# dkazanc/ToMoBAR

Hardware: AMD Instinct MI355X
Metric: fista_os_iterations_per_sec (higher is better)
Workload: dtype f32; 1 GPU; FISTA-OS(12 subsets)+PD_TV(30 inner, f32 duals), 900 angles, 1024 slices of 1024^2 per GPU; slab-iterations/s over 1 z-slab(s) (BASELINE configs[2]); slices_per_gpu=1024, n=1024, angles=900, os_number=12, method=FISTA, output_finite=True, input=analytic ellipsoid line integrals + Poisson noise (I0 2e4, peak attenuation 3), oversubscribed=False

## Files before the change

include/tomo_mi355x.h:

```cpp
#ifndef TOMO_MI355X_H
#define TOMO_MI355X_H

#include <stddef.h>
#include <stdint.h>

#ifdef __cplusplus
extern "C" {
#endif

#define TOMO_ABI_VERSION 10

enum {
    TOMO_OK = 0,
    TOMO_E_INVALID = 1,
    TOMO_E_RUNTIME = 2,
    TOMO_E_NOMEM = 3,
    TOMO_E_NODEVICE = 4
};

#define TOMO_FLAG_LERP8 1u

enum { TOMO_FID_LS = 0, TOMO_FID_PWLS = 1, TOMO_FID_KL = 2, TOMO_FID_RATIO = 3 };

typedef struct tomo_ctx tomo_ctx;

typedef struct {
    float cs, sn;
    float cor;
    float slope;
    float inv;
    float scale;
    int32_t dirx;
    int32_t src;
} tomo_angle_t;

int tomo_abi_version(void);
const char *tomo_build_flavour(void);
const char *tomo_last_error(void);
int tomo_device_count(int *count);

int tomo_ctx_create(int device, int nz, int n, int nu, int na, const double *angles_host,
                    const double *cor_host, int cor_stride, int os_number, unsigned flags,
                    tomo_ctx **out);
int tomo_ctx_destroy(tomo_ctx *ctx);
int tomo_ctx_os_number(const tomo_ctx *ctx);
int tomo_ctx_num_bins(const tomo_ctx *ctx);
int tomo_ctx_newind_table(const tomo_ctx *ctx, int64_t *out_host);
int tomo_ctx_subset_size(const tomo_ctx *ctx, int subset);
int tomo_ctx_angle_table(const tomo_ctx *ctx, int subset, tomo_angle_t *out_host, int capacity);
int tomo_ctx_release_scratch(tomo_ctx *ctx);
const char *tomo_ctx_kernel_path(const tomo_ctx *ctx, const char *op);

int tomo_fp3d(tomo_ctx *ctx, int subset, const float *vol_dev, float *sino_dev, void *stream);
int tomo_bp3d(tomo_ctx *ctx, int subset, const float *sino_dev, float *vol_dev, void *stream);

#define TOMO_GATHERED_B 1
#define TOMO_GATHERED_W 2
int tomo_fp3d_residual(tomo_ctx *ctx, int subset, const float *vol_dev, const float *b_dev,
                       const float *w_dev, int gathered, int fidelity, float *res_dev, void *stream);

enum { TOMO_ROBUST_NONE = 0, TOMO_ROBUST_HUBER = 1, TOMO_ROBUST_STUDENTST = 2 };
int tomo_fp3d_residual_robust(tomo_ctx *ctx, int subset, const float *vol_dev, const float *b_dev, const float *w_dev,
                              int gathered, int fidelity, int robust, float delta, float *res_dev, void *stream);
int tomo_sino_robust(float *res_dev, size_t count, int robust, float delta, void *stream);

int tomo_fp3d_residual_ring(tomo_ctx *ctx, int subset, const float *vol_dev, const float *b_full_dev,
                            const float *ring_dev, float ring_scale, float *res_dev, void *stream);
int tomo_ring_gh_reduce(float *res_dev, const float *w_full_dev, const int *src_dev, int nz, int na_s, int na_full,
                        int nu, const float *rx_dev, float l_inv, float *r_out_dev, void *stream);
int tomo_swls_apply(float *res_dev, const float *w_full_dev, const int *src_dev, int nz, int na_s, int na_full, int nu,
                    float beta, void *stream);
int tomo_ring_gh_update(float *r_dev, float *r_old_dev, float *rx_dev, float lambda, float beta, size_t count,
                        void *stream);

int tomo_shift_rows(const float *in_dev, float *out_dev, int nz, int na, int nu, const float *shift_dev, float sign,
                    void *stream);
int tomo_sino_residual(const float *ax_dev, const float *b_full_dev, const float *w_full_dev, const int *src_dev, int nz,
                       int na_s, int na_full, int nu, int gathered, int fidelity, float *res_dev, void *stream);
int tomo_sino_add_ring(float *res_dev, const float *ring_dev, float ring_scale, int nz, int na_s, int nu, void *stream);

int tomo_bp3d_fista(tomo_ctx *ctx, int subset, const float *res_dev, const float *xt_dev,
                    float *xout_dev, float l_inv, int nonneg, void *stream);
int tomo_bp3d_fista_momentum(tomo_ctx *ctx, int subset, const float *res_dev, float *xt_dev,
                             float *xold_x_dev, float l_inv, float beta, int nonneg, void *stream);
int tomo_bp3d_admm(tomo_ctx *ctx, int subset, const float *res_dev, float *z_dev, const float *x_dev,
                   const float *u_dev, float *zu_out_dev, float tau, float rho, int relax_on,
                   float one_minus_alpha, float alpha, int nonneg, void *stream);

int tomo_bp3d_matched(tomo_ctx *ctx, int subset, const float *sino_dev, float *vol_dev, void *stream);
int tomo_bp3d_matched_fista(tomo_ctx *ctx, int subset, const float *res_dev, const float *xt_dev,
                            float *xout_dev, float l_inv, int nonneg, void *stream);
int tomo_bp3d_matched_fista_momentum(tomo_ctx *ctx, int subset, const float *res_dev, float *xt_dev,
                                     float *xold_x_dev, float l_inv, float beta, int nonneg, void *stream);
int tomo_bp3d_matched_admm(tomo_ctx *ctx, int subset, const float *res_dev, float *z_dev, const float *x_dev,
                           const float *u_dev, float *zu_out_dev, float tau, float rho, int relax_on,
                           float one_minus_alpha, float alpha, int nonneg, void *stream);

enum { TOMO_RESIDUAL_PLANAR = 0, TOMO_RESIDUAL_ZQUAD = 1 };
int tomo_ctx_set_residual_layout(tomo_ctx *ctx, int layout);
int tomo_ctx_residual_layout(const tomo_ctx *ctx);
size_t tomo_ctx_residual_elems(const tomo_ctx *ctx, int subset);

int tomo_momentum(const float *x_dev, const float *xold_dev, float *xt_dev, float beta, size_t count, void *stream);
int tomo_momentum_transposed(tomo_ctx *ctx, const float *x_dev, const float *xold_dev, float *xt_dev, float beta,
                             void *stream);
int tomo_ctx_invalidate(tomo_ctx *ctx);
int tomo_admm_dual(float *u_dev, const float *z_dev, const float *x_dev, size_t count, void *stream);
int tomo_axpby(float a, const float *x_dev, float b, float *y_dev, size_t count, void *stream);
int tomo_scale(float a, const float *x_dev, float *y_dev, size_t count, void *stream);
int tomo_clamp_min(float *x_dev, float lo, size_t count, void *stream);
int tomo_mul(const float *x_dev, float *y_dev, size_t count, void *stream);
int tomo_recip_safe(const float *x_dev, float *y_dev, size_t count, void *stream);
int tomo_fill(float *x_dev, float value, size_t count, void *stream);
int tomo_norm2(const float *x_dev, size_t count, double *out_host, void *stream);
int tomo_dot(const float *x_dev, const float *y_dev, size_t count, double *out_host, void *stream);
int tomo_max(const float *x_dev, size_t count, float *out_host, void *stream);
int tomo_rel_change(const float *x_dev, const float *ref_dev, float *keep_dev, size_t count, double out_host[2], void *stream);
int tomo_pwls_weights(const float *b_dev, float *w_dev, size_t count, void *stream);
int tomo_pwls_max(const float *b_dev, size_t count, float *out_host, void *stream);
int tomo_pwls_weights_scaled(const float *b_dev, float *w_dev, size_t count, float wmax, void *stream);
int tomo_diag_stream(const float *const *in_dev, int nin, float *const *out_dev, int nout, size_t count,
                     int vec, int grid, void *stream);

int tomo_pad_edge(const float *in_dev, float *out_dev, int rows, int nu0, int pad, void *stream);
int tomo_crop_center(const float *in_dev, float *out_dev, int nz, int n, int m, void *stream);
int tomo_circ_mask(float *vol_dev, int nz, int n, double radius, void *stream);
int tomo_permute3(const float *in_dev, float *out_dev, int d0, int d1, int d2,
                  int64_t s0, int64_t s1, int64_t s2, void *stream);

int tomo_pdtv(int device, const float *in_dev, float *out_dev, int dx, int dy, int dz, int nd,
              float sigma, float tau, float lt, float theta, int iters, int methodTV, int nonneg,
              int half, void *stream);
int tomo_roftv(int device, const float *in_dev, float *out_dev, int dx, int dy, int dz, int nd,
               float lambda, float tau, int iters, int half, void *stream);
int tomo_pdtv_tol(int device, const float *in_dev, float *out_dev, int dx, int dy, int dz, int nd,
                  float sigma, float tau, float lt, float theta, int iters, int methodTV, int nonneg,
                  int half, double tol, int *iters_done, double *last_rel_change, void *stream);
int tomo_roftv_tol(int device, const float *in_dev, float *out_dev, int dx, int dy, int dz, int nd,
                   float lambda, float tau, int iters, int half, double tol, int *iters_done,
                   double *last_rel_change, void *stream);
int tomo_pdtv_slices(int device, const float *in_dev, float *out_dev, int dx, int dy, int nslices, float sigma,
                     float tau, float lt, float theta, int iters, int methodTV, int nonneg, int half, double tol,
                     int *iters_done, double *last_rel_change, void *stream);
int tomo_roftv_slices(int device, const float *in_dev, float *out_dev, int dx, int dy, int nslices, float lambda,
                      float tau, int iters, int half, double tol, int *iters_done, double *last_rel_change,
                      void *stream);
size_t tomo_pdtv_slices_scratch_bytes(int dx, int dy, int nslices, int half);
size_t tomo_roftv_slices_scratch_bytes(int dx, int dy, int nslices);
int tomo_tgv(int device, const float *in_dev, float *out_dev, int dx, int dy, int dz, int nd,
             float lambda, float alpha1, float alpha0, float tau, float sigma, int iters,
             double tol, int *iters_done, double *last_rel_change, void *stream);
enum { TOMO_NDF_HUBER = 0, TOMO_NDF_PM = 1, TOMO_NDF_TUKEY = 2 };
int tomo_ndf(int device, const float *in_dev, float *out_dev, int dx, int dy, int dz, int nd,
             float lambda, float sigma, float tau, int penalty, int iters,
             double tol, int *iters_done, double *last_rel_change, void *stream);
int tomo_diff4th(int device, const float *in_dev, float *out_dev, int dx, int dy, int dz, int nd,
                 float lambda, float sigma, float tau, int iters,
                 double tol, int *iters_done, double *last_rel_change, void *stream);
int tomo_llt_rof(int device, const float *in_dev, float *out_dev, int dx, int dy, int dz, int nd,
                 float lambda_rof, float lambda_llt, float tau, int iters,
                 double tol, int *iters_done, double *last_rel_change, void *stream);
size_t tomo_wavelet_scratch_bytes(int dx, int dy, int dz, int nd);
int tomo_wavelet_shrink(int device, const float *in_dev, float *out_dev, const float *mix_dev, int dx, int dy, int dz,
                        int nd, float threshold, void *stream);
int tomo_wavelet_forward(int device, const float *in_dev, float *pyramid_dev, int dx, int dy, int dz, int nd,
                         float threshold, void *stream);
int tomo_wavelet_inverse(int device, float *pyramid_dev, float *out_dev, const float *mix_dev, int dx, int dy, int dz,
                         int nd, void *stream);
size_t tomo_nltv_scratch_bytes(int dx, int dy, int dz, int nd);
int tomo_patch_select(int device, const float *in_dev, uint16_t *hi_dev, uint16_t *hj_dev, float *w_dev,
                      int dx, int dy, int dz, int nd, int search, int patch, int neighbours, float h, void *stream);
int tomo_nltv(int device, const float *in_dev, float *out_dev, const uint16_t *hi_dev, const uint16_t *hj_dev,
              const float *w_dev, int dx, int dy, int dz, int nd, int neighbours, float lambda, int iters,
              double tol, int *iters_done, double *last_rel_change, void *stream);
size_t tomo_pdtv_scratch_bytes(int dx, int dy, int dz, int nd, int half);
size_t tomo_roftv_scratch_bytes(int dx, int dy, int dz, int nd);
size_t tomo_tgv_scratch_bytes(int dx, int dy, int dz, int nd);
size_t tomo_ndf_scratch_bytes(int dx, int dy, int dz, int nd);
size_t tomo_diff4th_scratch_bytes(int dx, int dy, int dz, int nd);
size_t tomo_llt_rof_scratch_bytes(int dx, int dy, int dz, int nd);
int tomo_release_scratch(int device);
int tomo_reserve_scratch(int device, size_t bytes, void *stream);
int tomo_set_placement_tries(int tries);
int tomo_placement_tries(void);
int tomo_placed_scratch(int device, int slot, size_t bytes, void *stream, void **out_dev);
int tomo_placement_last(size_t *bytes, int *chosen, double *scores_GBps, int capacity);
int tomo_placement_last_fast(void);

int tomo_pdtv_iter_slab(int device, const float *in_dev, const float *u_in_dev, float *u_out_dev,
                        const void *p_in_dev[3], void *p_out_dev[3], int dx, int dy, int nz_local,
                        int has_lo, int has_hi, float sigma, float tau, float lt, float theta,
                        int methodTV, int nonneg, int half, void *stream);
int tomo_pdtv_multi_slab_range(int device, const float *in_dev, const float *u_in_dev, float *u_out_dev,
                               const void *p_in_dev[3], void *p_out_dev[3], int dx, int dy, int nz_local,
                               int lo_planes, int hi_planes, int z_begin, int z_end, int k, float sigma, float tau,
                               float lt, float theta, int methodTV, int nonneg, int half, void *stream);
int tomo_roftv_iter_slab_range(int device, const float *in_dev, const float *u_in_dev, float *u_out_dev,
                               int dx, int dy, int nz_local, int lo_planes, int hi_planes, int z_begin, int z_end,
                               float lambda, float tau, int half, void *stream);
int tomo_ndf_iter_slab_range(int device, const float *in_dev, const float *u_in_dev, float *u_out_dev,
                             int dx, int dy, int nz_local, int lo_planes, int hi_planes, int z_begin, int z_end,
                             float lambda, float sigma, float tau, int penalty, void *stream);
int tomo_diff4th_iter_slab_range(int device, const float *in_dev, const float *u_in_dev, float *u_out_dev,
                                 int dx, int dy, int nz_local, int lo_planes, int hi_planes, int z_begin, int z_end,
                                 float lambda, float sigma, float tau, void *stream);
int tomo_llt_rof_iter_slab_range(int device, const float *in_dev, const float *u_in_dev, float *u_out_dev,
                                 int dx, int dy, int nz_local, int lo_planes, int hi_planes, int z_begin, int z_end,
                                 float lambda_rof, float lambda_llt, float tau, void *stream);

size_t tomo_halo_staging_bytes(const size_t *bytes, int nblocks);
int tomo_halo_pack(const void *const *src_dev, const size_t *bytes, int nblocks, void *staging_dev, void *stream);
int tomo_halo_unpack(const void *staging_dev, void *const *dst_dev, const size_t *bytes, int nblocks, void *stream);
int tomo_halo_pack2(const void *const *src_down_dev, const size_t *bytes_down, int nblocks_down, void *msg_down_dev,
                    const void *const *src_up_dev, const size_t *bytes_up, int nblocks_up, void *msg_up_dev, void *stream);
int tomo_halo_pull2(const void *msg_down_dev, void *const *dst_down_dev, const size_t *bytes_down, int nblocks_down,
                    const void *msg_up_dev, void *const *dst_up_dev, const size_t *bytes_up, int nblocks_up, void *stream);
int tomo_ipc_region_create(int device, size_t bytes, void **base_dev, unsigned char handle[64]);
int tomo_ipc_region_open(int device, const unsigned char handle[64], void **mapped_dev);
int tomo_ipc_region_close(void *mapped_dev);
int tomo_ipc_region_destroy(void *base_dev);
int tomo_pdtv_iters_per_launch(int half);
int tomo_pdtv_launch_plan(int iters, int nd, int dz, int *k_out, int capacity);

int tomo_fbp_filter(int device, float *data_dev, size_t rows, int nu, float cutoff, float multiplier, void *stream);

int tomo_fourier_inv(int device, const float *data_dev, float *out_dev, int nz, int out_z, int nproj, int raw_n,
                     int n, int ne, int unpad_m, int out_size, const float *w_host, const float *theta_host,
                     int m, float mu, int center_size, void *stream);

int tomo_set_variant(const char *kernel, int variant);

int tomo_profile_enable(int on);
int tomo_profile_read(const char *kernel, long long *launches, double *total_ms);

int tomo_host_bp2d(const float *sino_host, float *img_host, int n, int nu, int na, const double *angles_host, double cor);
int tomo_host_fp2d(const float *img_host, float *sino_host, int n, int nu, int na, const double *angles_host, double cor);

#ifdef __cplusplus
}
#endif
#endif
```

tomobar_amd/_lib.py:

```python

from __future__ import annotations

import contextvars
import ctypes as C
import os
import threading

_HERE = os.path.dirname(os.path.abspath(__file__))
LIB_PATH = os.path.join(_HERE, "libtomo_mi355x.so")

OK, E_INVALID, E_RUNTIME, E_NOMEM, E_NODEVICE = 0, 1, 2, 3, 4
ABI_VERSION = 10
FLAG_LERP8 = 1
FID = {"LS": 0, "PWLS": 1, "KL": 2, "RATIO": 3}
ROBUST = {None: 0, "huber": 1, "studentst": 2}
RESIDUAL_LAYOUT = {"planar": 0, "zquad": 1}
NDF_PENALTY = {"Huber": 0, "PM": 1, "Tukey": 2}


def ndf_penalty_id(penalty_type) -> int:
    if penalty_type not in NDF_PENALTY:
        raise ValueError(f"unknown NDF penalty {penalty_type!r}: Huber, PM and Tukey are supported")
    return NDF_PENALTY[penalty_type]


class AngleRecord(C.Structure):
    _fields_ = [("cs", C.c_float), ("sn", C.c_float), ("cor", C.c_float), ("slope", C.c_float),
                ("inv", C.c_float), ("scale", C.c_float), ("dirx", C.c_int32), ("src", C.c_int32)]


_vp, _i, _f, _d, _sz = C.c_void_p, C.c_int, C.c_float, C.c_double, C.c_size_t

SIGNATURES = {
    "tomo_abi_version": (_i, []),
    "tomo_build_flavour": (C.c_char_p, []),
    "tomo_last_error": (C.c_char_p, []),
    "tomo_device_count": (_i, [C.POINTER(_i)]),
    "tomo_ctx_create": (_i, [_i, _i, _i, _i, _i, C.POINTER(_d), C.POINTER(_d), _i, _i, C.c_uint, C.POINTER(_vp)]),
    "tomo_ctx_destroy": (_i, [_vp]),
    "tomo_ctx_os_number": (_i, [_vp]),
    "tomo_ctx_num_bins": (_i, [_vp]),
    "tomo_ctx_newind_table": (_i, [_vp, C.POINTER(C.c_int64)]),
    "tomo_ctx_subset_size": (_i, [_vp, _i]),
    "tomo_ctx_angle_table": (_i, [_vp, _i, C.POINTER(AngleRecord), _i]),
    "tomo_ctx_release_scratch": (_i, [_vp]),
    "tomo_ctx_kernel_path": (C.c_char_p, [_vp, C.c_char_p]),
    "tomo_fp3d": (_i, [_vp, _i, _vp, _vp, _vp]),
    "tomo_bp3d": (_i, [_vp, _i, _vp, _vp, _vp]),
    "tomo_fp3d_residual": (_i, [_vp, _i, _vp, _vp, _vp, _i, _i, _vp, _vp]),
    "tomo_fp3d_residual_robust": (_i, [_vp, _i, _vp, _vp, _vp, _i, _i, _i, _f, _vp, _vp]),
    "tomo_sino_robust": (_i, [_vp, _sz, _i, _f, _vp]),
    "tomo_fp3d_residual_ring": (_i, [_vp, _i, _vp, _vp, _vp, _f, _vp, _vp]),
    "tomo_ring_gh_reduce": (_i, [_vp, _vp, _vp, _i, _i, _i, _i, _vp, _f, _vp, _vp]),
    "tomo_swls_apply": (_i, [_vp, _vp, _vp, _i, _i, _i, _i, _f, _vp]),
    "tomo_ring_gh_update": (_i, [_vp, _vp, _vp, _f, _f, _sz, _vp]),
    "tomo_shift_rows": (_i, [_vp, _vp, _i, _i, _i, _vp, _f, _vp]),
    "tomo_sino_add_ring": (_i, [_vp, _vp, _f, _i, _i, _i, _vp]),
    "tomo_sino_residual": (_i, [_vp, _vp, _vp, _vp, _i, _i, _i, _i, _i, _i, _vp, _vp]),
    "tomo_bp3d_fista": (_i, [_vp, _i, _vp, _vp, _vp, _f, _i, _vp]),
    "tomo_bp3d_fista_momentum": (_i, [_vp, _i, _vp, _vp, _vp, _f, _f, _i, _vp]),
    "tomo_bp3d_admm": (_i, [_vp, _i, _vp, _vp, _vp, _vp, _vp, _f, _f, _i, _f, _f, _i, _vp]),
    "tomo_bp3d_matched": (_i, [_vp, _i, _vp, _vp, _vp]),
    "tomo_bp3d_matched_fista": (_i, [_vp, _i, _vp, _vp, _vp, _f, _i, _vp]),
    "tomo_bp3d_matched_fista_momentum": (_i, [_vp, _i, _vp, _vp, _vp, _f, _f, _i, _vp]),
    "tomo_bp3d_matched_admm": (_i, [_vp, _i, _vp, _vp, _vp, _vp, _vp, _f, _f, _i, _f, _f, _i, _vp]),
    "tomo_ctx_set_residual_layout": (_i, [_vp, _i]),
    "tomo_ctx_residual_layout": (_i, [_vp]),
    "tomo_ctx_residual_elems": (_sz, [_vp, _i]),
    "tomo_momentum": (_i, [_vp, _vp, _vp, _f, _sz, _vp]),
    "tomo_momentum_transposed": (_i, [_vp, _vp, _vp, _vp, _f, _vp]),
    "tomo_ctx_invalidate": (_i, [_vp]),
    "tomo_admm_dual": (_i, [_vp, _vp, _vp, _sz, _vp]),
    "tomo_axpby": (_i, [_f, _vp, _f, _vp, _sz, _vp]),
    "tomo_scale": (_i, [_f, _vp, _vp, _sz, _vp]),
    "tomo_clamp_min": (_i, [_vp, _f, _sz, _vp]),
    "tomo_mul": (_i, [_vp, _vp, _sz, _vp]),
    "tomo_recip_safe": (_i, [_vp, _vp, _sz, _vp]),
    "tomo_fill": (_i, [_vp, _f, _sz, _vp]),
    "tomo_norm2": (_i, [_vp, _sz, C.POINTER(_d), _vp]),
    "tomo_dot": (_i, [_vp, _vp, _sz, C.POINTER(_d), _vp]),
    "tomo_max": (_i, [_vp, _sz, C.POINTER(_f), _vp]),
    "tomo_rel_change": (_i, [_vp, _vp, _vp, _sz, C.POINTER(_d), _vp]),
    "tomo_pwls_weights": (_i, [_vp, _vp, _sz, _vp]),
    "tomo_pwls_max": (_i, [_vp, _sz, C.POINTER(_f), _vp]),
    "tomo_pwls_weights_scaled": (_i, [_vp, _vp, _sz, _f, _vp]),
    "tomo_diag_stream": (_i, [C.POINTER(_vp), _i, C.POINTER(_vp), _i, _sz, _i, _i, _vp]),
    "tomo_pad_edge": (_i, [_vp, _vp, _i, _i, _i, _vp]),
    "tomo_crop_center": (_i, [_vp, _vp, _i, _i, _i, _vp]),
    "tomo_circ_mask": (_i, [_vp, _i, _i, _d, _vp]),
    "tomo_permute3": (_i, [_vp, _vp, _i, _i, _i, C.c_int64, C.c_int64, C.c_int64, _vp]),
    "tomo_pdtv": (_i, [_i, _vp, _vp, _i, _i, _i, _i, _f, _f, _f, _f, _i, _i, _i, _i, _vp]),
    "tomo_roftv": (_i, [_i, _vp, _vp, _i, _i, _i, _i, _f, _f, _i, _i, _vp]),
    "tomo_pdtv_tol": (_i, [_i, _vp, _vp, _i, _i, _i, _i, _f, _f, _f, _f, _i, _i, _i, _i, _d, C.POINTER(_i), C.POINTER(_d), _vp]),
    "tomo_roftv_tol": (_i, [_i, _vp, _vp, _i, _i, _i, _i, _f, _f, _i, _i, _d, C.POINTER(_i), C.POINTER(_d), _vp]),
    "tomo_pdtv_scratch_bytes": (_sz, [_i, _i, _i, _i, _i]),
    "tomo_roftv_scratch_bytes": (_sz, [_i, _i, _i, _i]),
    "tomo_pdtv_slices": (_i, [_i, _vp, _vp, _i, _i, _i, _f, _f, _f, _f, _i, _i, _i, _i, _d, C.POINTER(_i), C.POINTER(_d), _vp]),
    "tomo_roftv_slices": (_i, [_i, _vp, _vp, _i, _i, _i, _f, _f, _i, _i, _d, C.POINTER(_i), C.POINTER(_d), _vp]),
    "tomo_pdtv_slices_scratch_bytes": (_sz, [_i, _i, _i, _i]),
    "tomo_roftv_slices_scratch_bytes": (_sz, [_i, _i, _i]),
    "tomo_tgv": (_i, [_i, _vp, _vp, _i, _i, _i, _i, _f, _f, _f, _f, _f, _i, _d, C.POINTER(_i), C.POINTER(_d), _vp]),
    "tomo_tgv_scratch_bytes": (_sz, [_i, _i, _i, _i]),
    "tomo_ndf": (_i, [_i, _vp, _vp, _i, _i, _i, _i, _f, _f, _f, _i, _i, _d, C.POINTER(_i), C.POINTER(_d), _vp]),
    "tomo_ndf_scratch_bytes": (_sz, [_i, _i, _i, _i]),
    "tomo_diff4th": (_i, [_i, _vp, _vp, _i, _i, _i, _i, _f, _f, _f, _i, _d, C.POINTER(_i), C.POINTER(_d), _vp]),
    "tomo_diff4th_scratch_bytes": (_sz, [_i, _i, _i, _i]),
    "tomo_llt_rof": (_i, [_i, _vp, _vp, _i, _i, _i, _i, _f, _f, _f, _i, _d, C.POINTER(_i), C.POINTER(_d), _vp]),
    "tomo_llt_rof_scratch_bytes": (_sz, [_i, _i, _i, _i]),
    "tomo_wavelet_scratch_bytes": (_sz, [_i, _i, _i, _i]),
    "tomo_wavelet_shrink": (_i, [_i, _vp, _vp, _vp, _i, _i, _i, _i, _f, _vp]),
    "tomo_wavelet_forward": (_i, [_i, _vp, _vp, _i, _i, _i, _i, _f, _vp]),
    "tomo_wavelet_inverse": (_i, [_i, _vp, _vp, _vp, _i, _i, _i, _i, _vp]),
    "tomo_nltv_scratch_bytes": (_sz, [_i, _i, _i, _i]),
    "tomo_patch_select": (_i, [_i, _vp, _vp, _vp, _vp, _i, _i, _i, _i, _i, _i, _i, _f, _vp]),
    "tomo_nltv": (_i, [_i, _vp, _vp, _vp, _vp, _vp, _i, _i, _i, _i, _i, _f, _i, _d, C.POINTER(_i), C.POINTER(_d), _vp]),
    "tomo_release_scratch": (_i, [_i]),
    "tomo_reserve_scratch": (_i, [_i, _sz, _vp]),
    "tomo_set_placement_tries": (_i, [_i]),
    "tomo_placement_tries": (_i, []),
    "tomo_placement_last_fast": (_i, []),
    "tomo_placed_scratch": (_i, [_i, _i, _sz, _vp, C.POINTER(_vp)]),
    "tomo_placement_last": (_i, [C.POINTER(C.c_size_t), C.POINTER(_i), C.POINTER(C.c_double), _i]),
    "tomo_pdtv_iter_slab": (_i, [_i, _vp, _vp, _vp, C.POINTER(_vp), C.POINTER(_vp), _i, _i, _i, _i, _i,
                                 _f, _f, _f, _f, _i, _i, _i, _vp]),
    "tomo_pdtv_multi_slab_range": (_i, [_i, _vp, _vp, _vp, C.POINTER(_vp), C.POINTER(_vp), _i, _i, _i, _i, _i, _i, _i, _i,
                                        _f, _f, _f, _f, _i, _i, _i, _vp]),
    "tomo_roftv_iter_slab_range": (_i, [_i, _vp, _vp, _vp, _i, _i, _i, _i, _i, _i, _i, _f, _f, _i, _vp]),
    "tomo_ndf_iter_slab_range": (_i, [_i, _vp, _vp, _vp, _i, _i, _i, _i, _i, _i, _i, _f, _f, _f, _i, _vp]),
    "tomo_diff4th_iter_slab_range": (_i, [_i, _vp, _vp, _vp, _i, _i, _i, _i, _i, _i, _i, _f, _f, _f, _vp]),
    "tomo_llt_rof_iter_slab_range": (_i, [_i, _vp, _vp, _vp, _i, _i, _i, _i, _i, _i, _i, _f, _f, _f, _vp]),
    "tomo_halo_staging_bytes": (_sz, [C.POINTER(_sz), _i]),
    "tomo_halo_pack": (_i, [C.POINTER(_vp), C.POINTER(_sz), _i, _vp, _vp]),
    "tomo_halo_unpack": (_i, [_vp, C.POINTER(_vp), C.POINTER(_sz), _i, _vp]),
    "tomo_halo_pack2": (_i, [C.POINTER(_vp), C.POINTER(_sz), _i, _vp, C.POINTER(_vp), C.POINTER(_sz), _i, _vp, _vp]),
    "tomo_halo_pull2": (_i, [_vp, C.POINTER(_vp), C.POINTER(_sz), _i, _vp, C.POINTER(_vp), C.POINTER(_sz), _i, _vp]),
    "tomo_ipc_region_create": (_i, [_i, _sz, C.POINTER(_vp), C.POINTER(C.c_ubyte)]),
    "tomo_ipc_region_open": (_i, [_i, C.POINTER(C.c_ubyte), C.POINTER(_vp)]),
    "tomo_ipc_region_close": (_i, [_vp]),
    "tomo_ipc_region_destroy": (_i, [_vp]),
    "tomo_pdtv_iters_per_launch": (_i, [_i]),
    "tomo_pdtv_launch_plan": (_i, [_i, _i, _i, C.POINTER(_i), _i]),
    "tomo_fbp_filter": (_i, [_i, _vp, _sz, _i, _f, _f, _vp]),
    "tomo_fourier_inv": (_i, [_i, _vp, _vp, _i, _i, _i, _i, _i, _i, _i, _i, _vp, _vp, _i, _f, _i, _vp]),
    "tomo_host_bp2d": (_i, [_vp, _vp, _i, _i, _i, C.POINTER(_d), _d]),
    "tomo_host_fp2d": (_i, [_vp, _vp, _i, _i, _i, C.POINTER(_d), _d]),
    "tomo_set_variant": (_i, [C.c_char_p, _i]),
    "tomo_profile_enable": (_i, [_i]),
    "tomo_profile_read": (_i, [C.c_char_p, C.POINTER(C.c_longlong), C.POINTER(_d)]),
}

LIB_PATHS = {"shipped": LIB_PATH, "dev": os.path.join(_HERE, "libtomo_mi355x_dev.so")}
_handles = {}
_DEFAULT_FLAVOUR = "dev" if os.environ.get("TOMO_MI355X_FLAVOUR", "shipped") == "dev" else "shipped"
_flavour_var = contextvars.ContextVar("tomo_mi355x_flavour", default=_DEFAULT_FLAVOUR)


class TomoRuntimeError(RuntimeError):
    pass


def _load(flavour: str):
    path = LIB_PATHS[flavour]
    if not os.path.exists(path):
        raise ImportError(
            f"{path} not found: the HIP extension is required (no CPU fallback). "
            f"Build it with `make -C tomobar_amd/csrc{' dev' if flavour == 'dev' else ''}` or `__graft_entry__.build()`.")
    handle = C.CDLL(path)
    missing = [name for name in SIGNATURES if not hasattr(handle, name)]
    if missing:
        raise ImportError(f"{path} is stale: it does not export {missing[:4]}{'...' if len(missing) > 4 else ''}; "
                          "rebuild it (make -C tomobar_amd/csrc all)")
    for name, (res, args) in SIGNATURES.items():
        fn = getattr(handle, name)
        fn.restype = res
        fn.argtypes = args
    if handle.tomo_abi_version() != ABI_VERSION:
        raise ImportError(f"{os.path.basename(path)} has ABI version {handle.tomo_abi_version()}, this package binds "
                          f"version {ABI_VERSION}: rebuild it (make -C tomobar_amd/csrc all)")
    if handle.tomo_build_flavour().decode() != flavour:
        raise ImportError(f"{path} reports flavour {handle.tomo_build_flavour().decode()!r}, expected {flavour!r}")
    return handle


_load_lock = threading.Lock()


def lib():
    name = _flavour_var.get()
    h = _handles.get(name)
    if h is None:
        with _load_lock:
            h = _handles.get(name)
            if h is None:
                h = _handles[name] = _load(name)
    return h


def flavour() -> str:
    return _flavour_var.get()


class use_flavour:

    def __init__(self, name: str):
        if name not in LIB_PATHS:
            raise ValueError(f"unknown library flavour {name!r}")
        self.name = name
        self._token = None

    def __enter__(self):
        self._token = _flavour_var.set(self.name)
        return lib()

    def __exit__(self, *exc):
        if self._token is not None:
            _flavour_var.reset(self._token)
            self._token = None
        return False

    enter, exit = __enter__, __exit__


def check(rc: int, handle=None):
    if rc == OK:
        return
    msg = (handle or lib()).tomo_last_error().decode("utf-8", "replace")
    if rc == E_INVALID:
        raise ValueError(msg)
    if rc == E_NOMEM:
        raise MemoryError(msg)
    raise TomoRuntimeError(msg)
```

tomobar_amd/csrc/proj_kernels.hip:

```cpp
#include "tomo_common.h"

#include <algorithm>
#include <atomic>
#include <cmath>
#include <map>
#include <mutex>
#include <numeric>
#include <string>
#include <type_traits>

namespace {

template <bool LERP8>
__device__ __forceinline__ float lerp_w(float f, float fl)
{
    float w = f - fl;
    if (LERP8) w = rintf(w * 256.0f) * (1.0f / 256.0f);
    return w;
}

__device__ __forceinline__ float robust_weight(float r, int mode, float delta)
{
    if (mode == TOMO_ROBUST_HUBER) {
        const float ar = fabsf(r);
        if (ar > delta) r = (delta / ar) * r;
    } else if (mode == TOMO_ROBUST_STUDENTST) {
        r = (2.0f / (delta * delta + r * r)) * r;
    }
    return r;
}

enum { EPI_PLAIN = 0, EPI_FISTA = 1, EPI_FISTA_MOM = 2, EPI_ADMM = 3 };

struct BpArgs {
    const float *sino;
    int zquad;
    const tomo_angle_t *tab;
    int nz, n, nu, na;
    float *vol;
    const float *xt;
    float *xout;
    float *xt_out;
    const float *xold;
    float s0, s1, s2, s3;
    int nonneg, relax_on;
    int ntx, nty, nzb;
    int epi_aligned;
    int device;
    std::string *path;
};

template <int EPI>
__device__ __forceinline__ void bp_epilogue(const BpArgs &a, size_t idx, float g)
{
    if (EPI == EPI_PLAIN) {
        a.vol[idx] = g;
    } else if (EPI == EPI_FISTA) {
        float x = a.xt[idx] - a.s0 * g;
        if (a.nonneg) x = x < 0.0f ? 0.0f : x;
        a.xout[idx] = x;
    } else if (EPI == EPI_FISTA_MOM) {
        float x = a.xt[idx] - a.s0 * g;
        if (a.nonneg) x = x < 0.0f ? 0.0f : x;
        const float xo = a.xold[idx];
        a.xout[idx] = x;
        a.xt_out[idx] = x + a.s1 * (x - xo);
    } else {
        const float z0 = a.xout[idx], u = a.xold[idx];
        const float ga = a.s1 * ((z0 - a.xt[idx]) + u);
        float z = z0 - a.s0 * (g + ga);
        if (a.nonneg) z = z < 0.0f ? 0.0f : z;
        if (a.relax_on) z = a.s2 * z0 + a.s3 * z;
        a.xout[idx] = z;
        a.xt_out[idx] = z + u;
    }
}

template <int EPI>
__device__ __forceinline__ void bp_epilogue4(const BpArgs &a, size_t idx, float4 g)
{
#ifndef TOMO_BP_EPI_TEMPORAL
    typedef float v4 __attribute__((ext_vector_type(4)));
    auto ld4 = [&](const float *p) {
        const v4 t = __builtin_nontemporal_load(reinterpret_cast<const v4 *>(p + idx));
        return make_float4(t.x, t.y, t.z, t.w);
    };
    auto st4 = [&](float *p, float4 v) { __builtin_nontemporal_store(v4{v.x, v.y, v.z, v.w}, reinterpret_cast<v4 *>(p + idx)); };
#else
    auto ld4 = [&](const float *p) { return *reinterpret_cast<const float4 *>(p + idx); };
    auto st4 = [&](float *p, float4 v) { *reinterpret_cast<float4 *>(p + idx) = v; };
#endif
    const float gv[4] = {g.x, g.y, g.z, g.w};
    if (EPI == EPI_PLAIN) {
        st4(a.vol, g);
    } else if (EPI == EPI_FISTA) {
        const float4 t4 = ld4(a.xt);
        const float tv[4] = {t4.x, t4.y, t4.z, t4.w};
        float o[4];
#pragma unroll
        for (int k = 0; k < 4; ++k) {
            float x = tv[k] - a.s0 * gv[k];
            if (a.nonneg) x = x < 0.0f ? 0.0f : x;
            o[k] = x;
        }
        st4(a.xout, make_float4(o[0], o[1], o[2], o[3]));
    } else if (EPI == EPI_FISTA_MOM) {
        const float4 t4 = ld4(a.xt), o4 = ld4(a.xold);
        const float tv[4] = {t4.x, t4.y, t4.z, t4.w}, ov[4] = {o4.x, o4.y, o4.z, o4.w};
        float o[4], m[4];
#pragma unroll
        for (int k = 0; k < 4; ++k) {
            float x = tv[k] - a.s0 * gv[k];
            if (a.nonneg) x = x < 0.0f ? 0.0f : x;
            o[k] = x;
            m[k] = x + a.s1 * (x - ov[k]);
        }
        st4(a.xout, make_float4(o[0], o[1], o[2], o[3]));
        st4(a.xt_out, make_float4(m[0], m[1], m[2], m[3]));
    } else {
        const float4 z4 = ld4(a.xout), u4 = ld4(a.xold), t4 = ld4(a.xt);
        const float zv[4] = {z4.x, z4.y, z4.z, z4.w}, uv[4] = {u4.x, u4.y, u4.z, u4.w}, tv[4] = {t4.x, t4.y, t4.z, t4.w};
        float o[4], m[4];
#pragma unroll
        for (int k = 0; k < 4; ++k) {
            const float ga = a.s1 * ((zv[k] - tv[k]) + uv[k]);
            float z = zv[k] - a.s0 * (gv[k] + ga);
            if (a.nonneg) z = z < 0.0f ? 0.0f : z;
            if (a.relax_on) z = a.s2 * zv[k] + a.s3 * z;
            o[k] = z;
            m[k] = z + uv[k];
        }
        st4(a.xout, make_float4(o[0], o[1], o[2], o[3]));
        st4(a.xt_out, make_float4(m[0], m[1], m[2], m[3]));
    }
}

template <int EPI, bool LERP8>
__global__ __launch_bounds__(256) void bp_direct_kernel(BpArgs a)
{
    constexpr int ZB = 4;
    const int ix = blockIdx.x * 64 + (threadIdx.x & 63);
    const int iy = blockIdx.y * 4 + (threadIdx.x >> 6);
    const int z0 = blockIdx.z * ZB;
    if (ix >= a.n || iy >= a.n) return;
    const float half_n = 0.5f * (float)a.n - 0.5f, half_u = 0.5f * (float)a.nu - 0.5f;
    const float xw = (float)ix - half_n, yw = (float)iy - half_n;
    float acc[ZB] = {0.0f, 0.0f, 0.0f, 0.0f};
    const size_t zstride = (size_t)a.na * a.nu;
    for (int k = 0; k < a.na; ++k) {
        const tomo_angle_t t = a.tab[k];
        const float off = half_u - t.cor;
        const float f = fmaf(xw, t.cs, fmaf(yw, t.sn, off));
        const float fl = floorf(f);
        const float w = lerp_w<LERP8>(f, fl), omw = 1.0f - w;
        const int i0 = (int)fl;
        const bool ok0 = (i0 >= 0) && (i0 < a.nu), ok1 = (i0 + 1 >= 0) && (i0 + 1 < a.nu);
        if (a.zquad) {
            const float4 *row4 = reinterpret_cast<const float4 *>(a.sino) + ((size_t)(z0 >> 2) * a.na + k) * a.nu;
            const float4 zero4 = make_float4(0.0f, 0.0f, 0.0f, 0.0f);
            const float4 q0 = ok0 ? row4[i0] : zero4, q1 = ok1 ? row4[i0 + 1] : zero4;
            const float t0[ZB] = {q0.x, q0.y, q0.z, q0.w}, t1[ZB] = {q1.x, q1.y, q1.z, q1.w};
#pragma unroll
            for (int zz = 0; zz < ZB; ++zz) {
                acc[zz] = fmaf(omw, t0[zz], acc[zz]);
                acc[zz] = fmaf(w, t1[zz], acc[zz]);
            }
            continue;
        }
        const float *row = a.sino + ((size_t)z0 * a.na + k) * a.nu;
#pragma unroll
        for (int zz = 0; zz < ZB; ++zz) {
            const bool zok = z0 + zz < a.nz;
            const float s0 = (ok0 && zok) ? row[zz * zstride + i0] : 0.0f;
            const float s1 = (ok1 && zok) ? row[zz * zstride + i0 + 1] : 0.0f;
            acc[zz] = fmaf(omw, s0, acc[zz]);
            acc[zz] = fmaf(w, s1, acc[zz]);
        }
    }
#pragma unroll
    for (int zz = 0; zz < ZB; ++zz)
        if (z0 + zz < a.nz) bp_epilogue<EPI>(a, ((size_t)(z0 + zz) * a.n + iy) * a.n + ix, acc[zz]);
}

constexpr int BP_TX = 64, BP_TY = 8, BP_RY = 2, BP_ZQ = 4, BP_AB = 8, BP_PITCH = 72;

template <int EPI, bool LERP8>
__global__ __launch_bounds__(256) void bp_tiled_kernel(BpArgs a)
{
    __shared__ float4 tile[BP_AB][BP_ZQ][BP_PITCH];
    __shared__ int umin_s[BP_AB];

    const int ntiles = a.ntx * a.nty;
    const int b = blockIdx.x, xcd = b & 7, q = b >> 3;
    const int per_xcd = (a.nzb * ntiles + 7) >> 3;
    const int wi = xcd * per_xcd + q;
    if (wi >= a.nzb * ntiles) return;
    const int zb = wi / ntiles;
    const int tid = wi % ntiles;
    const int tx0 = (tid % a.ntx) * BP_TX, ty0 = (tid / a.ntx) * BP_TY;
    const int z0 = zb * (4 * BP_ZQ);

    const int lane = threadIdx.x & 63, wave = threadIdx.x >> 6;
    const int ix = tx0 + lane;
    const float half_n = 0.5f * (float)a.n - 0.5f, half_u = 0.5f * (float)a.nu - 0.5f;
    const float xw = (float)ix - half_n;
    float yw[BP_RY];
#pragma unroll
    for (int r = 0; r < BP_RY; ++r) yw[r] = (float)(ty0 + wave * BP_RY + r) - half_n;

    float acc[BP_RY][4 * BP_ZQ];
#pragma unroll
    for (int r = 0; r < BP_RY; ++r)
#pragma unroll
        for (int j = 0; j < 4 * BP_ZQ; ++j) acc[r][j] = 0.0f;

    const size_t zstride = (size_t)a.na * a.nu;
    for (int a0 = 0; a0 < a.na; a0 += BP_AB) {
        const int nb = min(BP_AB, a.na - a0);
        __syncthreads();
        if ((int)threadIdx.x < nb) {
            const tomo_angle_t t = a.tab[a0 + threadIdx.x];
            const float off = half_u - t.cor;
            const float x0 = (float)tx0 - half_n, x1 = (float)(tx0 + BP_TX - 1) - half_n;
            const float y0 = (float)ty0 - half_n, y1 = (float)(ty0 + BP_TY - 1) - half_n;
            const float f00 = fmaf(x0, t.cs, fmaf(y0, t.sn, off)), f10 = fmaf(x1, t.cs, fmaf(y0, t.sn, off));
            const float f01 = fmaf(x0, t.cs, fmaf(y1, t.sn, off)), f11 = fmaf(x1, t.cs, fmaf(y1, t.sn, off));
            umin_s[threadIdx.x] = (int)floorf(fminf(fminf(f00, f10), fminf(f01, f11)));
        }
        __syncthreads();
        for (int item = threadIdx.x; item < nb * BP_ZQ * BP_PITCH; item += 256) {
            const int j = item % BP_PITCH;
            const int zq = (item / BP_PITCH) % BP_ZQ;
            const int aa = item / (BP_PITCH * BP_ZQ);
            const int u = umin_s[aa] + j;
            float4 v = make_float4(0.0f, 0.0f, 0.0f, 0.0f);
            if (u >= 0 && u < a.nu) {
                const int z = z0 + zq * 4;
                const float *p = a.sino + ((size_t)z * a.na + (a0 + aa)) * a.nu + u;
                if (z + 0 < a.nz) v.x = p[0];
                if (z + 1 < a.nz) v.y = p[zstride];
                if (z + 2 < a.nz) v.z = p[2 * zstride];
                if (z + 3 < a.nz) v.w = p[3 * zstride];
            }
            tile[aa][zq][j] = v;
        }
        __syncthreads();
        for (int aa = 0; aa < nb; ++aa) {
            const tomo_angle_t t = a.tab[a0 + aa];
            const float off = half_u - t.cor;
            const int um = umin_s[aa];
#pragma unroll
            for (int r = 0; r < BP_RY; ++r) {
                const float f = fmaf(xw, t.cs, fmaf(yw[r], t.sn, off));
                const float fl = floorf(f);
                const float w = lerp_w<LERP8>(f, fl), omw = 1.0f - w;
                const int idx = (int)fl - um;
#pragma unroll
                for (int zq = 0; zq < BP_ZQ; ++zq) {
                    const float4 s0 = tile[aa][zq][idx];
                    const float4 s1 = tile[aa][zq][idx + 1];
                    float *c = &acc[r][zq * 4];
                    c[0] = fmaf(omw, s0.x, c[0]); c[0] = fmaf(w, s1.x, c[0]);
                    c[1] = fmaf(omw, s0.y, c[1]); c[1] = fmaf(w, s1.y, c[1]);
                    c[2] = fmaf(omw, s0.z, c[2]); c[2] = fmaf(w, s1.z, c[2]);
                    c[3] = fmaf(omw, s0.w, c[3]); c[3] = fmaf(w, s1.w, c[3]);
                }
            }
        }
    }
    if (ix < a.n) {
#pragma unroll
        for (int r = 0; r < BP_RY; ++r) {
            const int iy = ty0 + wave * BP_RY + r;
            if (iy < a.n) {
#pragma unroll
                for (int j = 0; j < 4 * BP_ZQ; ++j)
                    if (z0 + j < a.nz) bp_epilogue<EPI>(a, ((size_t)(z0 + j) * a.n + iy) * a.n + ix, acc[r][j]);
            }
        }
    }
}

#include "bp_brick.inl"

__global__ __launch_bounds__(256) void sino_to_quad_kernel(const float *__restrict__ in, float4 *__restrict__ out, int nz, size_t row)
{
    const size_t i = (size_t)blockIdx.x * 256 + threadIdx.x;
    const int z = 4 * (int)blockIdx.y;
    if (i >= row) return;
    const float *p = in + (size_t)z * row + i;
    float4 v;
    v.x = p[0];
    v.y = z + 1 < nz ? p[row] : 0.0f;
    v.z = z + 2 < nz ? p[2 * row] : 0.0f;
    v.w = z + 3 < nz ? p[3 * row] : 0.0f;
    out[(size_t)blockIdx.y * row + i] = v;
}

constexpr size_t BP_RELAY_MAX_BYTES = (size_t)16 << 30;
constexpr int BP_RELAY_DEVICES = 64, BP_RELAY_RETRY = 64;
struct bp_relay_state { std::atomic<size_t> refused{~(size_t)0}; std::atomic<unsigned> skipped{0}; };
bp_relay_state g_bp_relay[BP_RELAY_DEVICES];

template <int EPI>
int bp_launch(BpArgs a, bool lerp8, hipStream_t st)
{
    TOMO_ON_DEVICE(a.device);
    tomo_prof_scope prof(PROF_BP, st, 1);
    {
        uintptr_t bits = 0;
        if (EPI == EPI_PLAIN) bits |= (uintptr_t)a.vol;
        else bits |= (uintptr_t)a.xt | (uintptr_t)a.xout;
        if (EPI == EPI_FISTA_MOM || EPI == EPI_ADMM) bits |= (uintptr_t)a.xt_out | (uintptr_t)a.xold;
        a.epi_aligned = (bits & 15) == 0;
    }
    if (EPI == EPI_PLAIN) a.zquad = 0;
    if (a.zquad && (((uintptr_t)a.sino) & 15) != 0)
        return tomo_fail(TOMO_E_INVALID, "the quad-interleaved residual must be 16-byte aligned");
    bool relaid = false;
    if (g_variant_bp == 0 && !a.zquad && (long)a.na * a.nu < (1L << 25) && a.na > 0) {
        const size_t row = (size_t)a.na * a.nu, nq = (size_t)ceil_div(a.nz, 4), bytes = nq * row * 16;
        void *q = nullptr;
        bp_relay_state &rs = g_bp_relay[a.device >= 0 && a.device < BP_RELAY_DEVICES ? a.device : 0];
        bool have = bytes <= BP_RELAY_MAX_BYTES && nq <= 65535;
        if (have && bytes >= rs.refused.load() && (rs.skipped.fetch_add(1) + 1) % BP_RELAY_RETRY != 0) have = false;
        if (have) {
            const int rc = tomo_arena_get(a.device, st, ARENA_BPQ, bytes, &q);
            if (rc == TOMO_E_NOMEM) {
                rs.refused.store(std::min(rs.refused.load(), bytes));
                tomo_warn_once("bp_relay", "back projection: no memory for the quad-interleaved relay of a planar sinogram, "
                                           "running the planar staging (slower; asked again every 64th call and after tomo_release_scratch)");
                have = false;
            } else if (rc != TOMO_OK) {
                return rc;
            } else {
                rs.refused.store(~(size_t)0);
            }
        }
        if (have) {
            sino_to_quad_kernel<<<dim3((unsigned)((row + 255) / 256), (unsigned)nq), 256, 0, st>>>(a.sino, (float4 *)q, a.nz, row);
            TOMO_LAUNCH_CHECK();
            a.sino = (const float *)q;
            a.zquad = 1;
            relaid = true;
        }
    }
    const bool brick_ok = (long)a.na * a.nu < (a.zquad ? (1L << 25) : (1L << 27));
    const int variant = g_variant_bp == 3 ? 0 : g_variant_bp;
    if (variant == 1 || (variant == 0 && !brick_ok)) {
        if (variant == 0)
            tomo_warn_once("bp_direct", "back projection: angles x detector >= 2^27 samples per slice, falling back to "
                                        "the direct (no LDS) kernel (about 3.5x slower)");
        if (a.path) *a.path = "direct(no LDS)";
        dim3 grid(ceil_div(a.n, 64), ceil_div(a.n, 4), ceil_div(a.nz, 4));
        if (lerp8) bp_direct_kernel<EPI, true><<<grid, 256, 0, st>>>(a);
        else bp_direct_kernel<EPI, false><<<grid, 256, 0, st>>>(a);
    } else if (variant == 0) {
        if (a.path) *a.path = "brick(32x16x16)";
        a.ntx = ceil_div(a.n, BB_TX);
        a.nty = ceil_div(a.n, BB_TY);
        a.nzb = ceil_div(a.nz, 4 * BB_ZQ);
        const long blocks = 8L * (((long)a.nzb * a.ntx * a.nty + 7) / 8);
        if (blocks > 0x7fffffffL) return tomo_fail(TOMO_E_INVALID, "volume too large for one BP launch");
        if (a.zquad) {
            if (a.path) *a.path = relaid ? "brick(32x16x16, planar sinogram re-laid quad-interleaved, LDS-DMA staging)"
                                         : "brick(32x16x16, quad-interleaved residual, LDS-DMA staging)";
            if (lerp8) bp_brick_kernel<EPI, true, true><<<(unsigned)blocks, 256, 0, st>>>(a);
            else bp_brick_kernel<EPI, false, true><<<(unsigned)blocks, 256, 0, st>>>(a);
            TOMO_LAUNCH_CHECK();
            return TOMO_OK;
        }
        if (lerp8) bp_brick_kernel<EPI, true><<<(unsigned)blocks, 256, 0, st>>>(a);
        else bp_brick_kernel<EPI, false><<<(unsigned)blocks, 256, 0, st>>>(a);
    }
#if TOMO_DEV
    else {
        if (a.zquad) return tomo_fail(TOMO_E_INVALID, "bp variant 2 reads the planar residual layout only");
        if (a.path) *a.path = "tiled(64x8x16)";
        a.ntx = ceil_div(a.n, BP_TX);
        a.nty = ceil_div(a.n, BP_TY);
        a.nzb = ceil_div(a.nz, 4 * BP_ZQ);
        const long blocks = 8L * (((long)a.nzb * a.ntx * a.nty + 7) / 8);
        if (blocks > 0x7fffffffL) return tomo_fail(TOMO_E_INVALID, "volume too large for one BP launch");
        if (lerp8) bp_tiled_kernel<EPI, true><<<(unsigned)blocks, 256, 0, st>>>(a);
        else bp_tiled_kernel<EPI, false><<<(unsigned)blocks, 256, 0, st>>>(a);
    }
#endif
    TOMO_LAUNCH_CHECK();
    return TOMO_OK;
}

struct FpArgs {
    const float *vol;
    const float *volT;
    const tomo_angle_t *tab;
    int nz, n, nu, na, na_full;
    float *out;
    const float *b;
    const float *w;
    const float *ring;
    float ring_scale;
    int fidelity;
    int gathered;
    int zquad;
    int robust;
    float rdelta;
};

template <class Args>
__device__ __forceinline__ float fp_residual_value(const Args &a, float val, int z, int k_a, int src, int iu)
{
    const size_t gi = ((size_t)z * a.na + k_a) * a.nu + iu;
    const size_t fi = ((size_t)z * a.na_full + src) * a.nu + iu;
    const float bv = a.b[(a.gathered & TOMO_GATHERED_B) ? gi : fi];
    if (a.fidelity == TOMO_FID_KL || a.fidelity == TOMO_FID_RATIO) {
        const float ax = val < 1e-8f ? 1e-8f : val;
        const float q = bv / ax;
        return (a.fidelity == TOMO_FID_KL) ? 1.0f - q : q;
    }
    val = val - bv;
    if (a.ring) val = val + a.ring_scale * a.ring[(size_t)z * a.nu + iu];
    if (a.w) val = val * a.w[(a.gathered & TOMO_GATHERED_W) ? gi : fi];
    return robust_weight(val, a.robust, a.rdelta);
}

__global__ __launch_bounds__(256) void transpose_inplane_kernel(const float *__restrict__ in, float *__restrict__ out, int n)
{
    __shared__ float t[32][33];
    const size_t zoff = (size_t)blockIdx.z * n * n;
    const int bx = blockIdx.x * 32, by = blockIdx.y * 32;
    const int lx = threadIdx.x & 31, ly = threadIdx.x >> 5;
    for (int r = ly; r < 32; r += 8) {
        const int x = bx + lx, y = by + r;
        t[r][lx] = (x < n && y < n) ? in[zoff + (size_t)y * n + x] : 0.0f;
    }
    __syncthreads();
    for (int r = ly; r < 32; r += 8) {
        const int y = by + lx, x = bx + r;
        if (x < n && y < n) out[zoff + (size_t)x * n + y] = t[lx][r];
    }
}

__global__ __launch_bounds__(256) void momentum_transpose_kernel(const float *__restrict__ x, const float *__restrict__ xold,
                                                                float *__restrict__ xt, float *__restrict__ xt_T, float beta, int n)
{
    __shared__ float t[32][33];
    const size_t zoff = (size_t)blockIdx.z * n * n;
    const int bx = blockIdx.x * 32, by = blockIdx.y * 32;
    const int lx = threadIdx.x & 31, ly = threadIdx.x >> 5;
    for (int r = ly; r < 32; r += 8) {
        const int xx = bx + lx, yy = by + r;
        float v = 0.0f;
        if (xx < n && yy < n) {
            const size_t i = zoff + (size_t)yy * n + xx;
            const float a = x[i];
            v = a + beta * (a - xold[i]);
            xt[i] = v;
        }
        t[r][lx] = v;
    }
    __syncthreads();
    for (int r = ly; r < 32; r += 8) {
        const int yy = by + lx, xx = bx + r;
        if (xx < n && yy < n) xt_T[zoff + (size_t)xx * n + yy] = t[lx][r];
    }
}

typedef float glue_v4 __attribute__((ext_vector_type(4)));
__device__ __forceinline__ float4 nt_ld4(const float *p)
{
    const glue_v4 v = __builtin_nontemporal_load(reinterpret_cast<const glue_v4 *>(p));
    return make_float4(v.x, v.y, v.z, v.w);
}
__device__ __forceinline__ void nt_st4(float *p, float4 v)
{
    __builtin_nontemporal_store(glue_v4{v.x, v.y, v.z, v.w}, reinterpret_cast<glue_v4 *>(p));
}
template <bool MOMENTUM>
__global__ __launch_bounds__(256) void transpose64_kernel(const float *__restrict__ x, const float *__restrict__ xold,
                                                          float *__restrict__ xt, float *__restrict__ xt_T, float beta, int n)
{
    __shared__ float t[64][65];
    const size_t zoff = (size_t)blockIdx.z * n * n;
    const int bx = blockIdx.x * 64, by = blockIdx.y * 64;
    const int c4 = (threadIdx.x & 15) * 4, r0 = threadIdx.x >> 4;
#pragma unroll
    for (int k = 0; k < 4; ++k) {
        const int r = r0 + 16 * k;
        const int xx = bx + c4, yy = by + r;
        float4 v = make_float4(0.0f, 0.0f, 0.0f, 0.0f);
        if (xx < n && yy < n) {
            const size_t i = zoff + (size_t)yy * n + xx;
            const float4 a = nt_ld4(x + i);
            if (MOMENTUM) {
                const float4 o = nt_ld4(xold + i);
                v.x = a.x + beta * (a.x - o.x); v.y = a.y + beta * (a.y - o.y);
                v.z = a.z + beta * (a.z - o.z); v.w = a.w + beta * (a.w - o.w);
                nt_st4(xt + i, v);
            } else {
                v = a;
            }
        }
        t[r][c4] = v.x; t[r][c4 + 1] = v.y; t[r][c4 + 2] = v.z; t[r][c4 + 3] = v.w;
    }
    __syncthreads();
#pragma unroll
    for (int k = 0; k < 4; ++k) {
        const int r = r0 + 16 * k;
        const int xx = bx + r, yy = by + c4;
        if (xx < n && yy < n)
            nt_st4(xt_T + zoff + (size_t)xx * n + yy, make_float4(t[c4][r], t[c4 + 1][r], t[c4 + 2][r], t[c4 + 3][r]));
    }
}

static inline bool aligned16(const void *a, const void *b, const void *c, const void *d)
{
#ifdef TOMO_GLUE32
    return false;
#endif
    return ((reinterpret_cast<uintptr_t>(a) | reinterpret_cast<uintptr_t>(b) | reinterpret_cast<uintptr_t>(c) | reinterpret_cast<uintptr_t>(d)) & 15) == 0;
}

template <bool LERP8, bool RESID>
__global__ __launch_bounds__(256) void fp_march_kernel(FpArgs a)
{
    constexpr int ZB = 4;
    const int iu = blockIdx.x * 256 + threadIdx.x;
    const int k_a = blockIdx.y;
    const int z0 = blockIdx.z * ZB;
    if (iu >= a.nu) return;
    const tomo_angle_t t = a.tab[k_a];
    const float half_n = 0.5f * (float)a.n - 0.5f, half_u = 0.5f * (float)a.nu - 0.5f;
    const float s = ((float)iu - half_u) + t.cor;
    const float offset = fmaf(s, t.inv, half_n);
    const float *src = t.dirx ? a.volT : a.vol;
    const size_t zstride = (size_t)a.n * a.n;
    const int n = a.n;
    float acc[ZB] = {0.0f, 0.0f, 0.0f, 0.0f};
    const float *base = src + (size_t)z0 * zstride;
    bool zok[ZB];
#pragma unroll
    for (int zz = 0; zz < ZB; ++zz) zok[zz] = z0 + zz < a.nz;
#pragma unroll 2
    for (int k = 0; k < n; ++k) {
        const float kw = (float)k - half_n;
        const float f = fmaf(kw, t.slope, offset);
        const float fl = floorf(f);
        const float w = lerp_w<LERP8>(f, fl), omw = 1.0f - w;
        const int i0 = (int)fl;
        const bool ok0 = (i0 >= 0) && (i0 < n), ok1 = (i0 + 1 >= 0) && (i0 + 1 < n);
        const float *row = base + (size_t)k * n;
#pragma unroll
        for (int zz = 0; zz < ZB; ++zz) {
            const float v0 = (ok0 && zok[zz]) ? row[zz * zstride + i0] : 0.0f;
            const float v1 = (ok1 && zok[zz]) ? row[zz * zstride + i0 + 1] : 0.0f;
            acc[zz] = fmaf(omw, v0, acc[zz]);
            acc[zz] = fmaf(w, v1, acc[zz]);
        }
    }
    float v4[ZB] = {0.0f, 0.0f, 0.0f, 0.0f};
#pragma unroll
    for (int zz = 0; zz < ZB; ++zz) {
        if (!zok[zz]) continue;
        const int z = z0 + zz;
        float val = acc[zz] * t.scale;
        if (RESID) val = fp_residual_value(a, val, z, k_a, t.src, iu);
        v4[zz] = val;
        if (!(RESID && a.zquad)) a.out[((size_t)z * a.na + k_a) * a.nu + iu] = val;
    }
    if (RESID && a.zquad)
        reinterpret_cast<float4 *>(a.out)[((size_t)(z0 >> 2) * a.na + k_a) * a.nu + iu] = make_float4(v4[0], v4[1], v4[2], v4[3]);
}

#include "fp_tiled.inl"

int fp_scratch(tomo_ctx *ctx)
{
    const size_t need = (size_t)ctx->nz * ctx->n * ctx->n * sizeof(float);
    if (ctx->scratch_bytes < need) {
        ctx->volT_valid = false;
        if (ctx->scratch) { TOMO_HIP(hipDeviceSynchronize()); TOMO_HIP(hipFree(ctx->scratch)); ctx->scratch = nullptr; ctx->scratch_bytes = 0; }
        TOMO_HIP(hipMalloc(&ctx->scratch, need));
        ctx->scratch_bytes = need;
    }
    return TOMO_OK;
}


static double fp_bank_model(double s, int m, int bt)
{
    double total = 0.0;
    int cnt = 0;
    for (int ph = 0; ph < 8; ++ph) {
        const double x0 = 3.0 + ph * 0.91;
        for (int t0 = 0; t0 + 16 <= bt; t0 += 16 * 5) {
            int distinct[16], nd = 0, rows[16] = {0};
            for (int j = 0; j < 16; ++j) {
                const int slot = (int)std::floor(x0 + s * (double)((m * (t0 + j)) % bt));
                bool seen = false;
                for (int q = 0; q < nd; ++q) seen |= distinct[q] == slot;
                if (!seen) { distinct[nd++] = slot; ++rows[slot & 15]; }
            }
            int worst = 1;
            for (int r = 0; r < 16; ++r) worst = std::max(worst, rows[r]);
            total += worst;
            ++cnt;
        }
    }
    return cnt ? total / cnt : 1.0;
}

static int fp_lane_mult(double s, int bt)
{
    static std::mutex mu;
    static std::map<std::pair<int, int>, int> memo;
    const int key = (int)std::lround((std::min(std::max(s, 1.0), 1.4143) - 1.0) * 512.0);
    std::lock_guard<std::mutex> lock(mu);
    auto it = memo.find({bt, key});
    if (it != memo.end()) return it->second;
    const double sq = 1.0 + key / 512.0;
    int best_m = 1;
    double best = fp_bank_model(sq, 1, bt);
    for (int m = 3; m < 64; m += 2) {
        if (std::gcd(m, bt) != 1) continue;
        const double c = fp_bank_model(sq, m, bt);
        if (c < best - 1e-3) { best = c; best_m = m; }
    }
    memo[{bt, key}] = best_m;
    return best_m;
}

static int fp_window_bound(const tomo_angle_t *tab, const int *order, int n_class, int n, int nu, int tile = 256,
                           int group = FP_A)
{
    const float half_n = 0.5f * (float)n - 0.5f, half_u = 0.5f * (float)nu - 0.5f;
    int bound = 2;
    const int nut = ceil_div(nu, tile);
    for (int g = 0; g * group < n_class; ++g) {
        const int ng = std::min(group, n_class - g * group);
        for (int ut = 0; ut < nut; ++ut) {
            for (int e = 0; e < 2; ++e) {
                const float kw = (float)(e ? n - 1 : 0) - half_n;
                float fmin = 3.0e38f, fmax = -3.0e38f;
                for (int i = 0; i < ng; ++i) {
                    const tomo_angle_t &t = tab[order[g * group + i]];
                    const float o0 = std::fmaf(((float)(ut * tile) - half_u) + t.cor, t.inv, half_n);
                    const float o1 = std::fmaf(((float)(ut * tile + tile - 1) - half_u) + t.cor, t.inv, half_n);
                    const float f0 = std::fmaf(kw, t.slope, o0), f1 = std::fmaf(kw, t.slope, o1);
                    fmin = std::min(fmin, std::min(f0, f1));
                    fmax = std::max(fmax, std::max(f0, f1));
                }
                const double wdt = (double)std::floor(fmax) + 1.0 - (double)std::floor(fmin) + 1.0;
                bound = std::max(bound, (int)std::min(wdt, (double)n + 4.0));
            }
        }
    }
    return std::min(bound + 2, n + 4);
}

constexpr int FP_A16 = 16;
constexpr int FP_WIDE_MIN_NU = 128;
constexpr int FP_MULT_MIN_BT = 768;

static int fp_wide_tiles(int nu) { return ceil_div(nu, 1024); }
static int fp_wide_bt(int nu) { return std::min(1024, ceil_div(ceil_div(nu, fp_wide_tiles(nu)), 64) * 64); }

enum FpForm { FP_WHOLE_ROW, FP_DENSE16, FP_TILED, FP_TILED_SYNC };

struct FpLaunch {
    FpForm form;
    int cls;
    bool merged;
    size_t order_off;
    int n_angles;
    int wpitch;
    int threads;
    int passes, kc;
    int nut, ngroups;
    size_t lds;
    long blocks;
    bool mult;
};

struct FpPlan {
    bool march = false;
    int count = 0;
    FpLaunch l[4];
};

static long fp_blocks(int nz, int nut, int ngroups) { return 8L * (((long)ceil_div(nz, 4) * nut * ngroups + 7) / 8); }

static bool fp_plan_whole_row(const tomo_ctx *ctx, int variant, int cls, bool merged, size_t off, int nc, int wp,
                              double cost_tiles, FpLaunch &l)
{
    const int nut = fp_wide_tiles(ctx->nu), bt = fp_wide_bt(ctx->nu);
    const double cost_rows = (double)nut * ceil_div(nc, FP_A) * wp;
    const bool pays = cost_tiles >= 0.9 * cost_rows;
    const int passes = ceil_div(wp, bt);
    int kc = 4;
    const size_t tab = (size_t)ctx->n * 8;
    size_t lds = (size_t)2 * kc * wp * 16 + tab;
    if (passes <= 2) {
        if (lds > 160 * 1024) { kc = 2; lds = (size_t)2 * kc * wp * 16 + tab; }
    } else {
        kc = passes == 3 ? 2 : 1;
        while (kc > 1 && (size_t)kc * wp * 16 + tab > 160 * 1024) --kc;
        lds = (size_t)kc * wp * 16 + tab;
    }
    if (!(pays && passes <= 5 && lds <= 160 * 1024)) return false;
    const bool mult = bt >= FP_MULT_MIN_BT && (size_t)2 * bt * 16 <= lds - tab && variant != 4;
    l = {FP_WHOLE_ROW, cls, merged, off, nc, wp, bt, passes, kc, nut, ceil_div(nc, FP_A), lds,
         fp_blocks(ctx->nz, nut, ceil_div(nc, FP_A)), mult};
    return true;
}

static bool fp_plan_dense16(const tomo_ctx *ctx, const tomo_subset &s, int variant, int cls, size_t off, FpLaunch &l)
{
    const int nc = s.n_class[cls], wp = s.wbound16[cls];
    if (nc < 2 * FP_A16) return false;
    if (wp > 512) return false;
    const int passes = ceil_div(wp, 256);
    const int kc = passes == 1 ? 4 : 2;
    const size_t lds = (size_t)2 * kc * wp * 16 + (size_t)ctx->n * 8;
    if (lds > 64 * 1024) return false;
    const int nut = ceil_div(ctx->nu, 256), ngroups = ceil_div(nc, FP_A16);
    const long wgs = (long)ceil_div(ctx->nz, 4) * nut * ngroups;
    if (fp_blocks(ctx->nz, nut, ngroups) > 0x7fffffffL) return false;
    if (wgs < 4 * 768 && variant != 3) return false;
    l = {FP_DENSE16, cls, false, off, nc, wp, 256, passes, kc, nut, ngroups, lds, fp_blocks(ctx->nz, nut, ngroups), false};
    return true;
}

static FpLaunch fp_plan_tiled(const tomo_ctx *ctx, const tomo_subset &s, int variant, int cls, size_t off)
{
    const int nc = s.n_class[cls], wp = s.wbound[cls], nut = ceil_div(ctx->nu, 256), ngroups = ceil_div(nc, FP_A);
    const long blocks = fp_blocks(ctx->nz, nut, ngroups);
    const int passes = ceil_div(wp, 256);
    if (variant == 2 || wp > FP_MAX_WPITCH) {
        const int kc = std::max(1, std::min(8, 40000 / (wp * 16)));
        return {FP_TILED_SYNC, cls, false, off, nc, wp, 256, passes, kc, nut, ngroups, (size_t)kc * wp * 16, blocks, false};
    }
    const int m = passes <= 2 ? 8 : (passes == 5 ? 10 : 12);
    const int kc = m / passes;
    const size_t lds = (size_t)(passes <= 2 ? 2 : 1) * kc * wp * 16 + (size_t)ctx->n * 8;
    return {FP_TILED, cls, false, off, nc, wp, 256, passes, kc, nut, ngroups, lds, blocks, false};
}

static int fp_plan(const tomo_ctx *ctx, const tomo_subset &s, int variant, FpPlan &plan)
{
    constexpr double FP_DENSE16_PAYS = 0.75;
    plan = FpPlan();
    plan.march = variant == 1;
    for (int c = 0; c < 4; ++c) plan.march |= s.n_class[c] > 0 && s.wbound[c] > 4000;
    if (plan.march) return TOMO_OK;
    const int nu = ctx->nu;
    size_t off[4] = {s.table_offset};
    for (int c = 1; c < 4; ++c) off[c] = off[c - 1] + s.n_class[c - 1];
    bool done[4] = {false, false, false, false};
    for (int d = 0; d < 2 && (variant == 0 || variant == 3 || variant == 4) && nu >= FP_WIDE_MIN_NU; ++d) {
        const int c0 = 2 * d, c1 = c0 + 1, nc0 = s.n_class[c0], nc1 = s.n_class[c1], nc = nc0 + nc1;
        if (nc == 0) continue;
        FpLaunch e0, e1;
        bool take = (nc0 == 0 || fp_plan_dense16(ctx, s, variant, c0, off[c0], e0)) &&
                    (nc1 == 0 || fp_plan_dense16(ctx, s, variant, c1, off[c1], e1));
        if (take && variant != 3) {
            const double cost = (nc0 ? (double)e0.nut * e0.ngroups * e0.wpitch : 0.0) +
                                (nc1 ? (double)e1.nut * e1.ngroups * e1.wpitch : 0.0);
            const int nut_w = fp_wide_tiles(nu);
            const double rows = nu <= 1024 ? (double)nut_w * ceil_div(nc, FP_A) * s.wbound_wide[c0]
                                           : (double)nut_w * ceil_div(nc0, FP_A) * s.wbound_wide[c0] +
                                             (double)nut_w * ceil_div(nc1, FP_A) * s.wbound_wide[c1];
            take = cost <= FP_DENSE16_PAYS * rows;
        }
        if (take) {
            if (nc0) plan.l[plan.count++] = e0;
            if (nc1) plan.l[plan.count++] = e1;
            done[c0] = done[c1] = true;
            continue;
        }
        if (variant == 3) continue;
        const int nut = ceil_div(nu, 256);
        const double ct0 = (double)nut * ceil_div(nc0, FP_A) * s.wbound[c0];
        const double ct1 = (double)nut * ceil_div(nc1, FP_A) * s.wbound[c1];
        FpLaunch l;
        if (nu <= 1024) {
            if (fp_plan_whole_row(ctx, variant, c0, true, off[c0], nc, s.wbound_wide[c0], ct0 + ct1, l)) {
                plan.l[plan.count++] = l;
                done[c0] = done[c1] = true;
            }
        } else {
            for (int c = c0; c <= c1; ++c)
                if (s.n_class[c] > 0 && fp_plan_whole_row(ctx, variant, c, false, off[c], s.n_class[c], s.wbound_wide[c],
                                                          c == c0 ? ct0 : ct1, l)) {
                    plan.l[plan.count++] = l;
                    done[c] = true;
                }
        }
    }
    for (int c = 0; c < 4; ++c)
        if (s.n_class[c] > 0 && !done[c]) plan.l[plan.count++] = fp_plan_tiled(ctx, s, variant, c, off[c]);
    for (int i = 0; i < plan.count; ++i) {
        TOMO_REQUIRE(plan.l[i].blocks <= 0x7fffffffL, "problem too large for one FP launch");
        TOMO_REQUIRE(plan.l[i].form != FP_TILED_SYNC || plan.l[i].lds <= 64 * 1024,
                     "forward-projection window does not fit in LDS");
    }
    return TOMO_OK;
}

static std::string fp_path_text(const FpLaunch &l)
{
    const std::string cls = "class" + std::to_string(l.cls) + ":", passes = std::to_string(l.passes) + " passes";
    switch (l.form) {
    case FP_WHOLE_ROW:
        return std::string(l.cls >> 1 ? "x" : "y") + (l.merged ? "" : (l.cls & 1) ? "-" : "+") + ":whole-row(" +
               std::to_string(l.threads) + " threads, " + passes + ", " + std::to_string(l.kc) + " rows/chunk) ";
    case FP_DENSE16: return cls + "dense(256 pixels x 16 angles, " + passes + ") ";
    case FP_TILED: return cls + "tiled-pipelined(256 threads, " + passes + ") ";
    default: return cls + "tiled-sync(window " + std::to_string(l.wpitch) + ") ";
    }
}

template <bool L8, bool RES>
static void fp_launch(const FpLaunch &l, const FpTiledArgs &t, hipStream_t st)
{
    using Kernel = void (*)(FpTiledArgs);
    const int m = l.passes * l.kc;
    Kernel k;
    switch (l.form) {
    case FP_TILED_SYNC:
        fp_tiled_sync_kernel<L8, RES, 256, FP_A><<<(unsigned)l.blocks, 256, l.lds, st>>>(t, l.kc);
        return;
    case FP_WHOLE_ROW:
        if (l.passes == 1) k = fp_tiled_kernel<L8, RES, 1, 4, true, 1024>;
        else if (l.passes == 2 && m == 8) k = fp_tiled_kernel<L8, RES, 2, 8, true, 1024>;
        else if (l.passes == 2) k = fp_tiled_kernel<L8, RES, 2, 4, true, 1024>;
        else if (l.passes == 3 && m == 6) k = fp_tiled_kernel<L8, RES, 3, 6, false, 1024>;
        else if (l.passes == 3) k = fp_tiled_kernel<L8, RES, 3, 3, false, 1024>;
        else if (l.passes == 4) k = fp_tiled_kernel<L8, RES, 4, 4, false, 1024>;
        else k = fp_tiled_kernel<L8, RES, 5, 5, false, 1024>;
        (void)hipFuncSetAttribute(reinterpret_cast<const void *>(k), hipFuncAttributeMaxDynamicSharedMemorySize, (int)l.lds);
        break;
    case FP_DENSE16:
        if (l.passes == 1) k = fp_tiled_kernel<L8, RES, 1, 4, true, 256, FP_A16>;
        else k = fp_tiled_kernel<L8, RES, 2, 4, true, 256, FP_A16>;
        break;
    default:
        if (l.passes == 1) k = fp_tiled_kernel<L8, RES, 1, 8, true, 256>;
        else if (l.passes == 2) k = fp_tiled_kernel<L8, RES, 2, 8, true, 256>;
        else if (l.passes == 3) k = fp_tiled_kernel<L8, RES, 3, 12, false, 256>;
        else if (l.passes == 4) k = fp_tiled_kernel<L8, RES, 4, 12, false, 256>;
        else k = fp_tiled_kernel<L8, RES, 5, 10, false, 256>;
    }
    k<<<(unsigned)l.blocks, l.threads, l.lds, st>>>(t);
}

int fp_run(tomo_ctx *ctx, int subset, const float *vol, const float *b, const float *w, int gathered, int fidelity,
           float *out, void *stream, const float *ring = nullptr, float ring_scale = 0.0f, int zquad = 0,
           int robust = TOMO_ROBUST_NONE, float rdelta = 0.0f)
{
    TOMO_REQUIRE(ctx != nullptr, "ctx is NULL");
    TOMO_REQUIRE(vol != nullptr && out != nullptr, "NULL data pointer");
    TOMO_REQUIRE(subset < ctx->os, "subset %d out of range (OS_number %d)", subset, ctx->os);
    const tomo_subset &s = (subset < 0 || ctx->os == 1) ? ctx->subsets[0] : ctx->subsets[1 + subset];
    hipStream_t st = as_stream(stream);
    const bool ready = ctx->volT_valid && ctx->volT_of == vol && ctx->volT_stream == st && ctx->scratch != nullptr;
    ctx->volT_valid = false;
    ctx->volT_of = nullptr;
    if (s.size == 0) return TOMO_OK;
    TOMO_ON_DEVICE(ctx->device);
    FpArgs a;
    a.vol = vol;
    a.volT = nullptr;
    if (s.n_dirx > 0) {
        int rc = fp_scratch(ctx);
        if (rc != TOMO_OK) return rc;
        if (!ready) {
            if (ctx->n % 4 == 0 && aligned16(vol, ctx->scratch, nullptr, nullptr)) {
                dim3 tg(ceil_div(ctx->n, 64), ceil_div(ctx->n, 64), ctx->nz);
                transpose64_kernel<false><<<tg, 256, 0, st>>>(vol, nullptr, nullptr, (float *)ctx->scratch, 0.0f, ctx->n);
            } else {
                dim3 tg(ceil_div(ctx->n, 32), ceil_div(ctx->n, 32), ctx->nz);
                transpose_inplane_kernel<<<tg, 256, 0, st>>>(vol, (float *)ctx->scratch, ctx->n);
            }
            TOMO_LAUNCH_CHECK();
        }
        a.volT = (const float *)ctx->scratch;
    }
    a.tab = ctx->dev_table + s.table_offset;
    a.nz = ctx->nz; a.n = ctx->n; a.nu = ctx->nu; a.na = s.size; a.na_full = ctx->na;
    a.out = out; a.b = b; a.w = w; a.fidelity = fidelity; a.gathered = gathered;
    a.ring = ring; a.ring_scale = ring_scale;
    a.robust = (b != nullptr) ? robust : TOMO_ROBUST_NONE; a.rdelta = rdelta;
    a.zquad = (b != nullptr) ? zquad : 0;
    if (a.zquad && (((uintptr_t)out) & 15) != 0)
        return tomo_fail(TOMO_E_INVALID, "the quad-interleaved residual must be 16-byte aligned");
    tomo_prof_scope prof(PROF_FP, st, 1);
    ctx->last_fp_path.clear();
    const bool l8 = (ctx->flags & TOMO_FLAG_LERP8) != 0;
    FpPlan plan;
    const int rc = fp_plan(ctx, s, g_variant_fp, plan);
    if (rc != TOMO_OK) return rc;
    if (plan.march) {
        ctx->last_fp_path = "march(no LDS)";
        if (g_variant_fp != 1) tomo_warn_once("fp_march", "forward projection: a staged row window exceeds 64 KiB of LDS, "
                                              "falling back to the un-tiled march kernel (about 4x slower)");
        dim3 grid(ceil_div(ctx->nu, 256), s.size, ceil_div(ctx->nz, 4));
        if (b) {
            if (l8) fp_march_kernel<true, true><<<grid, 256, 0, st>>>(a);
            else fp_march_kernel<false, true><<<grid, 256, 0, st>>>(a);
        } else {
            if (l8) fp_march_kernel<true, false><<<grid, 256, 0, st>>>(a);
            else fp_march_kernel<false, false><<<grid, 256, 0, st>>>(a);
        }
        TOMO_LAUNCH_CHECK();
        return TOMO_OK;
    }
    FpTiledArgs t;
    t.tab = a.tab;
    t.nz = a.nz; t.n = a.n; t.nu = a.nu; t.na = a.na; t.na_full = a.na_full;
    t.out = out; t.b = b; t.w = w; t.fidelity = fidelity; t.gathered = gathered;
    t.ring = ring; t.ring_scale = ring_scale; t.zquad = a.zquad; t.robust = a.robust; t.rdelta = a.rdelta;
#if TOMO_DEV
    t.probe = g_probe;
#endif
    t.nzb = ceil_div(a.nz, 4);
    for (int i = 0; i < plan.count; ++i) {
        const FpLaunch &l = plan.l[i];
        t.src = (l.cls >> 1) ? a.volT : a.vol;
        t.order = ctx->dev_fp_order + l.order_off;
        t.mult = l.mult ? ctx->dev_fp_mult + l.order_off : nullptr;
        t.n_class = l.n_angles; t.wpitch = l.wpitch; t.nut = l.nut; t.bt = l.threads; t.ngroups = l.ngroups;
        if (b) { if (l8) fp_launch<true, true>(l, t, st); else fp_launch<false, true>(l, t, st); }
        else   { if (l8) fp_launch<true, false>(l, t, st); else fp_launch<false, false>(l, t, st); }
        TOMO_LAUNCH_CHECK();
        ctx->last_fp_path += fp_path_text(l);
    }
    return TOMO_OK;
}

int bp_prepare(tomo_ctx *ctx, int subset, const float *sino, BpArgs &a)
{
    TOMO_REQUIRE(ctx != nullptr, "ctx is NULL");
    TOMO_REQUIRE(subset < ctx->os, "subset %d out of range (OS_number %d)", subset, ctx->os);
    const tomo_subset &s = (subset < 0 || ctx->os == 1) ? ctx->subsets[0] : ctx->subsets[1 + subset];
    TOMO_REQUIRE(sino != nullptr || s.size == 0, "NULL sinogram pointer");
    a = BpArgs();
    a.device = ctx->device;
    a.path = &ctx->last_bp_path;
    a.sino = sino;
    a.tab = ctx->dev_table + s.table_offset;
    a.nz = ctx->nz; a.n = ctx->n; a.nu = ctx->nu; a.na = s.size;
    return TOMO_OK;
}

}

int fp_tables(tomo_ctx *ctx)
{
    const int n = ctx->n, nu = ctx->nu, bt = fp_wide_bt(nu);
    for (tomo_subset &s : ctx->subsets) {
        const tomo_angle_t *tab = ctx->host_table.data() + s.table_offset;
        const int *order = ctx->host_fp_order.data() + s.table_offset;
        for (int d = 0, off = 0; d < 2; ++d) {
            const int nc0 = s.n_class[2 * d], nc1 = s.n_class[2 * d + 1];
            for (int h = 0; h < 2; ++h) {
                const int c = 2 * d + h, nc = h ? nc1 : nc0, o = off + (h ? nc0 : 0);
                if (nc == 0) continue;
                s.wbound[c] = fp_window_bound(tab, order + o, nc, n, nu);
                s.wbound16[c] = fp_window_bound(tab, order + o, nc, n, nu, 256, FP_A16);
                if (nu > 1024) s.wbound_wide[c] = fp_window_bound(tab, order + o, nc, n, nu, bt);
            }
            if (nu <= 1024 && nc0 + nc1 > 0) s.wbound_wide[2 * d] = fp_window_bound(tab, order + off, nc0 + nc1, n, nu, bt);
            off += nc0 + nc1;
        }
    }
    if (bt < FP_MULT_MIN_BT) return TOMO_OK;
    std::vector<int> mult(ctx->host_fp_order.size(), 1);
    for (const tomo_subset &s : ctx->subsets)
        for (int i = 0; i < s.size; ++i) {
            const tomo_angle_t &rec = ctx->host_table[s.table_offset + ctx->host_fp_order[s.table_offset + i]];
            mult[s.table_offset + i] = fp_lane_mult(std::fabs((double)rec.inv), bt);
        }
    TOMO_HIP(hipMalloc((void **)&ctx->dev_fp_mult, std::max<size_t>(mult.size(), 1) * sizeof(int)));
    TOMO_HIP(hipMemcpy(ctx->dev_fp_mult, mult.data(), mult.size() * sizeof(int), hipMemcpyHostToDevice));
    return TOMO_OK;
}

void tomo_bp_relay_reset(int device)
{
    if (device < 0 || device >= BP_RELAY_DEVICES) return;
    g_bp_relay[device].refused.store(~(size_t)0);
    g_bp_relay[device].skipped.store(0);
}

extern "C" int tomo_fp3d(tomo_ctx *ctx, int subset, const float *vol_dev, float *sino_dev, void *stream)
{
    return fp_run(ctx, subset, vol_dev, nullptr, nullptr, 0, TOMO_FID_LS, sino_dev, stream);
}

extern "C" int tomo_fp3d_residual(tomo_ctx *ctx, int subset, const float *vol_dev, const float *b_full_dev,
                                  const float *w_full_dev, int gathered, int fidelity, float *res_dev, void *stream)
{
    TOMO_REQUIRE(b_full_dev != nullptr, "projection data pointer is NULL");
    TOMO_REQUIRE(fidelity == TOMO_FID_LS || fidelity == TOMO_FID_PWLS || fidelity == TOMO_FID_KL ||
                     fidelity == TOMO_FID_RATIO,
                 "data_fidelity should be LS, PWLS or KL");
    TOMO_REQUIRE(fidelity != TOMO_FID_PWLS || w_full_dev != nullptr, "PWLS needs the weights");
    return fp_run(ctx, subset, vol_dev, b_full_dev, fidelity == TOMO_FID_PWLS ? w_full_dev : nullptr, gathered,
                  fidelity, res_dev, stream, nullptr, 0.0f, ctx ? ctx->res_layout : 0);
}

extern "C" int tomo_fp3d_residual_robust(tomo_ctx *ctx, int subset, const float *vol_dev, const float *b_full_dev,
                                         const float *w_full_dev, int gathered, int fidelity, int robust, float delta,
                                         float *res_dev, void *stream)
{
    TOMO_REQUIRE(b_full_dev != nullptr, "projection data pointer is NULL");
    TOMO_REQUIRE(fidelity == TOMO_FID_LS || fidelity == TOMO_FID_PWLS, "the Huber / Student's-t re-weighting applies to the LS and PWLS residuals");
    TOMO_REQUIRE(fidelity != TOMO_FID_PWLS || w_full_dev != nullptr, "PWLS needs the weights");
    TOMO_REQUIRE(robust == TOMO_ROBUST_NONE || robust == TOMO_ROBUST_HUBER || robust == TOMO_ROBUST_STUDENTST, "unknown robust mode %d", robust);
    TOMO_REQUIRE(robust == TOMO_ROBUST_NONE || delta > 0.0f, "the Huber / Student's-t threshold must be positive");
    return fp_run(ctx, subset, vol_dev, b_full_dev, fidelity == TOMO_FID_PWLS ? w_full_dev : nullptr, gathered,
                  fidelity, res_dev, stream, nullptr, 0.0f, ctx ? ctx->res_layout : 0, robust, delta);
}

extern "C" int tomo_ctx_set_residual_layout(tomo_ctx *ctx, int layout)
{
    TOMO_REQUIRE(ctx != nullptr, "ctx is NULL");
    TOMO_REQUIRE(layout == TOMO_RESIDUAL_PLANAR || layout == TOMO_RESIDUAL_ZQUAD, "unknown residual layout %d", layout);
    ctx->res_layout = layout;
    return TOMO_OK;
}

extern "C" int tomo_ctx_residual_layout(const tomo_ctx *ctx) { return ctx ? ctx->res_layout : -1; }

extern "C" size_t tomo_ctx_residual_elems(const tomo_ctx *ctx, int subset)
{
    if (!ctx || subset >= ctx->os) return 0;
    const tomo_subset &s = (subset < 0 || ctx->os == 1) ? ctx->subsets[0] : ctx->subsets[1 + subset];
    const size_t nzr = ctx->res_layout == TOMO_RESIDUAL_ZQUAD ? (size_t)ceil_div(ctx->nz, 4) * 4 : (size_t)ctx->nz;
    return nzr * (size_t)s.size * (size_t)ctx->nu;
}

extern "C" int tomo_momentum_transposed(tomo_ctx *ctx, const float *x_dev, const float *xold_dev, float *xt_dev, float beta,
                                        void *stream)
{
    TOMO_REQUIRE(ctx != nullptr && x_dev && xold_dev && xt_dev, "NULL argument");
    TOMO_ON_DEVICE(ctx->device);
    int rc = fp_scratch(ctx);
    if (rc != TOMO_OK) return rc;
    if (ctx->n % 4 == 0 && aligned16(x_dev, xold_dev, xt_dev, ctx->scratch)) {
        dim3 tg(ceil_div(ctx->n, 64), ceil_div(ctx->n, 64), ctx->nz);
        transpose64_kernel<true><<<tg, 256, 0, as_stream(stream)>>>(x_dev, xold_dev, xt_dev, (float *)ctx->scratch, beta, ctx->n);
    } else {
        dim3 tg(ceil_div(ctx->n, 32), ceil_div(ctx->n, 32), ctx->nz);
        momentum_transpose_kernel<<<tg, 256, 0, as_stream(stream)>>>(x_dev, xold_dev, xt_dev, (float *)ctx->scratch, beta, ctx->n);
    }
    TOMO_LAUNCH_CHECK();
    ctx->volT_of = xt_dev;
    ctx->volT_stream = as_stream(stream);
    ctx->volT_valid = true;
    return TOMO_OK;
}

extern "C" int tomo_ctx_invalidate(tomo_ctx *ctx)
{
    TOMO_REQUIRE(ctx != nullptr, "ctx is NULL");
    ctx->volT_valid = false;
    ctx->volT_of = nullptr;
    return TOMO_OK;
}

extern "C" int tomo_fp3d_residual_ring(tomo_ctx *ctx, int subset, const float *vol_dev, const float *b_full_dev,
                                       const float *ring_dev, float ring_scale, float *res_dev, void *stream)
{
    TOMO_REQUIRE(b_full_dev != nullptr && ring_dev != nullptr, "projection data / ring offset pointer is NULL");
    TOMO_REQUIRE(ctx == nullptr || ctx->res_layout == TOMO_RESIDUAL_PLANAR,
                 "the ring-term residual is read by tomo_ring_gh_reduce in the planar layout: set TOMO_RESIDUAL_PLANAR first");
    return fp_run(ctx, subset, vol_dev, b_full_dev, nullptr, 0, TOMO_FID_LS, res_dev, stream, ring_dev, ring_scale);
}

extern "C" int tomo_bp3d(tomo_ctx *ctx, int subset, const float *sino_dev, float *vol_dev, void *stream)
{
    BpArgs a;
    int rc = bp_prepare(ctx, subset, sino_dev, a);
    if (rc != TOMO_OK) return rc;
    TOMO_REQUIRE(vol_dev != nullptr, "NULL volume pointer");
    a.vol = vol_dev;
    return bp_launch<EPI_PLAIN>(a, (ctx->flags & TOMO_FLAG_LERP8) != 0, as_stream(stream));
}

extern "C" int tomo_bp3d_fista(tomo_ctx *ctx, int subset, const float *res_dev, const float *xt_dev,
                               float *xout_dev, float l_inv, int nonneg, void *stream)
{
    BpArgs a;
    int rc = bp_prepare(ctx, subset, res_dev, a);
    if (rc != TOMO_OK) return rc;
    TOMO_REQUIRE(xt_dev && xout_dev, "NULL volume pointer");
    a.xt = xt_dev; a.xout = xout_dev; a.s0 = l_inv; a.nonneg = nonneg;
    a.zquad = ctx->res_layout == TOMO_RESIDUAL_ZQUAD;
    return bp_launch<EPI_FISTA>(a, (ctx->flags & TOMO_FLAG_LERP8) != 0, as_stream(stream));
}

extern "C" int tomo_bp3d_fista_momentum(tomo_ctx *ctx, int subset, const float *res_dev, float *xt_dev,
                                        float *xold_x_dev, float l_inv, float beta, int nonneg, void *stream)
{
    BpArgs a;
    int rc = bp_prepare(ctx, subset, res_dev, a);
    if (rc != TOMO_OK) return rc;
    TOMO_REQUIRE(xt_dev && xold_x_dev, "NULL volume pointer");
    a.xt = xt_dev; a.xt_out = xt_dev; a.xold = xold_x_dev; a.xout = xold_x_dev;
    a.s0 = l_inv; a.s1 = beta; a.nonneg = nonneg;
    a.zquad = ctx->res_layout == TOMO_RESIDUAL_ZQUAD;
    return bp_launch<EPI_FISTA_MOM>(a, (ctx->flags & TOMO_FLAG_LERP8) != 0, as_stream(stream));
}

extern "C" int tomo_bp3d_admm(tomo_ctx *ctx, int subset, const float *res_dev, float *z_dev, const float *x_dev,
                              const float *u_dev, float *zu_out_dev, float tau, float rho, int relax_on,
                              float one_minus_alpha, float alpha, int nonneg, void *stream)
{
    BpArgs a;
    int rc = bp_prepare(ctx, subset, res_dev, a);
    if (rc != TOMO_OK) return rc;
    TOMO_REQUIRE(z_dev && x_dev && u_dev && zu_out_dev, "NULL volume pointer");
    a.xt = x_dev; a.xout = z_dev; a.xt_out = zu_out_dev; a.xold = u_dev;
    a.s0 = tau; a.s1 = rho; a.s2 = one_minus_alpha; a.s3 = alpha;
    a.nonneg = nonneg; a.relax_on = relax_on;
    a.zquad = ctx->res_layout == TOMO_RESIDUAL_ZQUAD;
    return bp_launch<EPI_ADMM>(a, (ctx->flags & TOMO_FLAG_LERP8) != 0, as_stream(stream));
}
```

tomobar_amd/csrc/tomo_api.hip:

```cpp
#include "tomo_common.h"

#include <algorithm>
#include <cmath>
#include <cstdlib>
#include <cstring>
#include <initializer_list>
#include <map>
#include <mutex>
#include <new>
#include <string>
#include <ctime>

static thread_local char g_err[512] = "";

int tomo_fail(int code, const char *fmt, ...)
{
    va_list ap;
    va_start(ap, fmt);
    vsnprintf(g_err, sizeof(g_err), fmt, ap);
    va_end(ap);
    return code;
}

thread_local int g_variant_bp = 0, g_variant_fp = 0, g_variant_pdtv = 0, g_variant_roftv = 0;
#if TOMO_DEV
thread_local int g_probe = 0;
#endif

extern "C" int tomo_abi_version(void) { return TOMO_ABI_VERSION; }
extern "C" const char *tomo_build_flavour(void) { return TOMO_DEV ? "dev" : "shipped"; }
extern "C" const char *tomo_last_error(void) { return g_err; }

extern "C" int tomo_device_count(int *count)
{
    TOMO_REQUIRE(count != nullptr, "count is NULL");
    int n = 0;
    hipError_t e = hipGetDeviceCount(&n);
    if (e != hipSuccess || n == 0) {
        *count = 0;
        return tomo_fail(TOMO_E_NODEVICE, "no HIP device visible (%s); libtomo_mi355x has no CPU fallback",
                         e == hipSuccess ? "device count 0" : hipGetErrorString(e));
    }
    *count = n;
    return TOMO_OK;
}

extern "C" int tomo_set_variant(const char *kernel, int variant)
{
    TOMO_REQUIRE(kernel != nullptr, "kernel name is NULL");
    std::string k(kernel);
    auto allowed = [&](std::initializer_list<int> shipped, std::initializer_list<int> dev) {
        for (int v : shipped) if (v == variant) return true;
        if (TOMO_DEV) for (int v : dev) if (v == variant) return true;
        return false;
    };
    int *slot = nullptr;
    bool ok = false;
    if (k == "bp") { slot = &g_variant_bp; ok = allowed({0}, {1, 2, 3}); }
    else if (k == "fp") { slot = &g_variant_fp; ok = allowed({0}, {1, 2, 3, 4}); }
    else if (k == "pdtv") { slot = &g_variant_pdtv; ok = allowed({0, 22}, {1, 2, 3, 21, 31, 32}); }
    else if (k == "roftv") { slot = &g_variant_roftv; ok = allowed({0}, {1, 2, 3, 4}); }
#if TOMO_DEV
    else if (k == "probe") { g_probe = variant; return TOMO_OK; }
#endif
    else return tomo_fail(TOMO_E_INVALID, "unknown kernel '%s'%s", kernel,
                          (!TOMO_DEV && k == "probe") ? " (measurement switches exist in libtomo_mi355x_dev.so only)" : "");
    if (!ok) return tomo_fail(TOMO_E_INVALID, "variant %d of '%s' is not part of this library (%s flavour)%s", variant, kernel,
                              tomo_build_flavour(), TOMO_DEV ? "" : ": the A/B variants live in libtomo_mi355x_dev.so");
    *slot = variant;
    return TOMO_OK;
}

static tomo_angle_t make_angle(double theta, double cor, int src)
{
    tomo_angle_t t;
    const double c = std::cos(theta), s = std::sin(theta);
    t.cs = (float)c;
    t.sn = (float)s;
    t.cor = (float)cor;
    t.dirx = std::fabs(s) >= std::fabs(c) ? 1 : 0;
    if (t.dirx) {
        t.slope = (float)(-c / s);
        t.inv = (float)(1.0 / s);
        t.scale = (float)(1.0 / std::fabs(s));
    } else {
        t.slope = (float)(-s / c);
        t.inv = (float)(1.0 / c);
        t.scale = (float)(1.0 / std::fabs(c));
    }
    t.src = src;
    return t;
}

extern "C" int tomo_ctx_create(int device, int nz, int n, int nu, int na, const double *angles_host,
                               const double *cor_host, int cor_stride, int os_number, unsigned flags,
                               tomo_ctx **out)
{
    TOMO_REQUIRE(out != nullptr, "out is NULL");
    *out = nullptr;
    TOMO_REQUIRE(nu > 0, "The size of the horizontal detector cannot be negative or zero");
    TOMO_REQUIRE(nz > 0, "The size of the vertical detector cannot be negative or zero");
    TOMO_REQUIRE(n > 0, "The size of the reconstruction object cannot be zero");
    TOMO_REQUIRE(na > 0 && angles_host != nullptr, "The length of angles array cannot be zero");
    TOMO_REQUIRE(os_number > 0, "The number of ordered subsets cannot be negative or zero");
    TOMO_REQUIRE(cor_host != nullptr && cor_stride >= 0 && cor_stride <= 2, "bad centre-of-rotation argument");
    TOMO_REQUIRE(device >= 0, "The GPU device index must be >= 0");
    if (cor_stride == 2)
        for (int a = 0; a < na; ++a)
            TOMO_REQUIRE(cor_host[2 * a + 1] == 0.0,
                         "the context takes horizontal offsets only: apply the vertical component (angle %d) with "
                         "tomo_shift_rows around the projectors, as HipTools3D does", a);
    int ndev = 0;
    int rc = tomo_device_count(&ndev);
    if (rc != TOMO_OK) return rc;
    TOMO_REQUIRE(device < ndev, "device index %d out of range (%d devices)", device, ndev);
    TOMO_ON_DEVICE(device);

    tomo_ctx *ctx = new (std::nothrow) tomo_ctx();
    if (!ctx) return tomo_fail(TOMO_E_NOMEM, "out of host memory");
    ctx->device = device;
    ctx->nz = nz; ctx->n = n; ctx->nu = nu; ctx->na = na;
    ctx->os = os_number;
    ctx->flags = flags;
    ctx->bins = (int)std::ceil((double)na / (double)os_number);

    auto cor_of = [&](int a) { return cor_stride == 0 ? cor_host[0] : cor_host[(size_t)a * cor_stride]; };
    auto push_subset = [&](const std::vector<int64_t> &idx) {
        tomo_subset s;
        s.size = (int)idx.size();
        s.table_offset = ctx->host_table.size();
        for (int64_t a : idx) {
            ctx->host_table.push_back(make_angle(angles_host[a], cor_of((int)a), (int)a));
            s.n_dirx += ctx->host_table.back().dirx;
        }
        const tomo_angle_t *tab = ctx->host_table.data() + s.table_offset;
        std::vector<int> order[4];
        for (int i = 0; i < s.size; ++i) order[2 * tab[i].dirx + (tab[i].inv < 0.0f ? 1 : 0)].push_back(i);
        for (int c = 0; c < 4; ++c) {
            std::stable_sort(order[c].begin(), order[c].end(), [&](int p, int q) { return tab[p].slope < tab[q].slope; });
            s.n_class[c] = (int)order[c].size();
            ctx->host_fp_order.insert(ctx->host_fp_order.end(), order[c].begin(), order[c].end());
        }
        ctx->subsets.push_back(s);
    };
    std::vector<int64_t> all(na);
    for (int a = 0; a < na; ++a) all[a] = a;
    push_subset(all);
    ctx->newind.assign((size_t)os_number * ctx->bins, 0);
    for (int s = 0; s < os_number; ++s)
        for (int k = 0; k < ctx->bins; ++k) {
            int64_t a = (int64_t)s + (int64_t)k * os_number;
            if (a < na) ctx->newind[(size_t)s * ctx->bins + k] = a;
        }
    if (os_number > 1) {
        for (int s = 0; s < os_number; ++s) {
            std::vector<int64_t> idx(ctx->newind.begin() + (size_t)s * ctx->bins,
                                     ctx->newind.begin() + (size_t)(s + 1) * ctx->bins);
            if (idx[ctx->bins - 1] == 0) idx.pop_back();
            push_subset(idx);
        }
    }
    size_t bytes = ctx->host_table.size() * sizeof(tomo_angle_t);
    hipError_t e = hipMalloc((void **)&ctx->dev_table, bytes > 0 ? bytes : sizeof(tomo_angle_t));
    if (e == hipSuccess && bytes)
        e = hipMemcpy(ctx->dev_table, ctx->host_table.data(), bytes, hipMemcpyHostToDevice);
    if (e == hipSuccess) {
        const size_t ob = ctx->host_fp_order.size() * sizeof(int);
        e = hipMalloc((void **)&ctx->dev_fp_order, ob > 0 ? ob : sizeof(int));
        if (e == hipSuccess && ob)
            e = hipMemcpy(ctx->dev_fp_order, ctx->host_fp_order.data(), ob, hipMemcpyHostToDevice);
    }
    if (e != hipSuccess) {
        if (ctx->dev_table) (void)hipFree(ctx->dev_table);
        if (ctx->dev_fp_order) (void)hipFree(ctx->dev_fp_order);
        delete ctx;
        return tomo_fail(TOMO_E_RUNTIME, "angle table upload failed: %s", hipGetErrorString(e));
    }
    rc = fp_tables(ctx);
    if (rc != TOMO_OK) { tomo_ctx_destroy(ctx); return rc; }
    *out = ctx;
    return TOMO_OK;
}

extern "C" int tomo_ctx_destroy(tomo_ctx *ctx)
{
    if (!ctx) return TOMO_OK;
    tomo_device_guard guard(ctx->device);
    if (ctx->dev_table) (void)hipFree(ctx->dev_table);
    if (ctx->dev_fp_order) (void)hipFree(ctx->dev_fp_order);
    if (ctx->dev_fp_mult) (void)hipFree(ctx->dev_fp_mult);
    if (ctx->scratch) (void)hipFree(ctx->scratch);
    delete ctx;
    return TOMO_OK;
}

extern "C" int tomo_ctx_release_scratch(tomo_ctx *ctx)
{
    TOMO_REQUIRE(ctx != nullptr, "ctx is NULL");
    ctx->volT_valid = false;
    ctx->volT_of = nullptr;
    if (ctx->scratch) {
        TOMO_ON_DEVICE(ctx->device);
        TOMO_HIP(hipDeviceSynchronize());
        TOMO_HIP(hipFree(ctx->scratch));
        ctx->scratch = nullptr;
        ctx->scratch_bytes = 0;
    }
    return tomo_arena_release_slot(ctx->device, ARENA_BPQ);
}

void tomo_warn_once(const char *key, const char *msg)
{
    static std::mutex mu;
    static std::map<std::string, bool> seen;
    std::lock_guard<std::mutex> lk(mu);
    if (seen[key]) return;
    seen[key] = true;
    fprintf(stderr, "libtomo_mi355x warning: %s\n", msg);
}

extern "C" const char *tomo_ctx_kernel_path(const tomo_ctx *ctx, const char *op)
{
    if (!ctx || !op) return "";
    return std::string(op) == "bp" ? ctx->last_bp_path.c_str() : ctx->last_fp_path.c_str();
}

extern "C" int tomo_ctx_os_number(const tomo_ctx *ctx) { return ctx ? ctx->os : -1; }
extern "C" int tomo_ctx_num_bins(const tomo_ctx *ctx) { return ctx ? ctx->bins : -1; }

extern "C" int tomo_ctx_newind_table(const tomo_ctx *ctx, int64_t *out_host)
{
    TOMO_REQUIRE(ctx != nullptr && out_host != nullptr, "NULL argument");
    std::memcpy(out_host, ctx->newind.data(), ctx->newind.size() * sizeof(int64_t));
    return TOMO_OK;
}

static const tomo_subset *find_subset(const tomo_ctx *ctx, int subset)
{
    if (!ctx) return nullptr;
    if (subset < 0 || ctx->os == 1) return &ctx->subsets[0];
    if (subset >= ctx->os) return nullptr;
    return &ctx->subsets[1 + subset];
}

extern "C" int tomo_ctx_subset_size(const tomo_ctx *ctx, int subset)
{
    const tomo_subset *s = find_subset(ctx, subset);
    return s ? s->size : -1;
}

extern "C" int tomo_ctx_angle_table(const tomo_ctx *ctx, int subset, tomo_angle_t *out_host, int capacity)
{
    const tomo_subset *s = find_subset(ctx, subset);
    TOMO_REQUIRE(s != nullptr && out_host != nullptr, "bad subset %d", subset);
    TOMO_REQUIRE(capacity >= s->size, "capacity %d < subset size %d", capacity, s->size);
    std::memcpy(out_host, ctx->host_table.data() + s->table_offset, (size_t)s->size * sizeof(tomo_angle_t));
    return TOMO_OK;
}

struct arena_t { void *ptr = nullptr; size_t bytes = 0; };
struct arena_key {
    int device; hipStream_t stream; int slot;
    bool operator<(const arena_key &o) const
    {
        if (device != o.device) return device < o.device;
        if (stream != o.stream) return stream < o.stream;
        return slot < o.slot;
    }
};
static std::mutex g_arena_mu;
static std::map<arena_key, arena_t> g_arenas;

namespace {
__global__ __launch_bounds__(256) void place_probe_kernel(const float *__restrict__ a, float *__restrict__ b, int nz, int zchunk)
{
    const int n = 1024, gx = 8, gy = 64;
    const int tile = (int)blockIdx.x % (gx * gy), chunk = (int)blockIdx.x / (gx * gy);
    const int xb = tile % gx, yb = tile / gx;
    const int lane = threadIdx.x & 63, wave = threadIdx.x >> 6;
    const int x = xb * 128 + (wave & 1) * 64 + lane, y0 = yb * 16 + (wave >> 1) * 8;
    const int z1 = min((chunk + 1) * zchunk, nz);
    for (int z = chunk * zchunk; z < z1; ++z) {
        const size_t pl = (size_t)z * n * n;
        float s = 0.0f;
#pragma unroll
        for (int r = -3; r < 11; ++r) s += a[pl + (size_t)min(max(y0 + r, 0), n - 1) * n + x];
#pragma unroll
        for (int r = 0; r < 8; ++r) b[pl + (size_t)(y0 + r) * n + x] = s;
    }
}
constexpr size_t PLACE_MIN_BYTES = (size_t)1 << 30;
constexpr size_t PLACE_HEADROOM = (size_t)4 << 30;
constexpr double PLACE_HOLD_FRACTION = 0.85;
constexpr int PLACE_MAX_TRIES = 10;
constexpr int PLACE_DEFAULT_TRIES = 8;
constexpr double PLACE_FAST_GAIN = 1.08;
int g_place_tries = -1;
struct place_rec { size_t bytes = 0; int tries = 0, chosen = -1, fast = 0; double score[PLACE_MAX_TRIES] = {0}; } g_place_last;
std::mutex g_place_mu;

int placement_tries()
{
    if (g_place_tries < 0) {
        const char *e = std::getenv("TOMO_MI355X_PLACE_TRIES");
        const int v = e ? std::atoi(e) : PLACE_DEFAULT_TRIES;
        g_place_tries = v < 1 ? 1 : (v > PLACE_MAX_TRIES ? PLACE_MAX_TRIES : v);
    }
    return g_place_tries;
}

double place_score(void *p, size_t bytes, hipStream_t st)
{
    const int nz = (int)(bytes / 2 / ((size_t)4 << 20));
    if (nz < 16) return 0.0;
    const int chunks = 16, zchunk = (nz + chunks - 1) / chunks;
    const float *a = (const float *)p;
    float *b = (float *)((char *)p + (size_t)nz * ((size_t)4 << 20));
    hipEvent_t e[3];
    int made = 0;
    for (; made < 3; ++made)
        if (hipEventCreateWithFlags(&e[made], hipEventDefault) != hipSuccess) break;
    double best = 0.0;
    bool ok = made == 3;
    if (ok) {
        place_probe_kernel<<<512 * chunks, 256, 0, st>>>(a, b, nz, zchunk);
        ok = hipGetLastError() == hipSuccess;
    }
    for (int r = 0; r < 2 && ok; ++r) {
        ok = hipEventRecord(e[r], st) == hipSuccess;
        place_probe_kernel<<<512 * chunks, 256, 0, st>>>(a, b, nz, zchunk);
        ok = ok && hipGetLastError() == hipSuccess;
        ok = ok && hipEventRecord(e[r + 1], st) == hipSuccess && hipEventSynchronize(e[r + 1]) == hipSuccess;
        float ms = 0.0f;
        ok = ok && hipEventElapsedTime(&ms, e[r], e[r + 1]) == hipSuccess && ms > 0.0f;
        if (ok) best = std::max(best, 2.0 * nz * (double)((size_t)4 << 20) / ms / 1e6);
    }
    for (int k = 0; k < made; ++k) (void)hipEventDestroy(e[k]);
    if (!ok) (void)hipGetLastError();
    return ok ? best : 0.0;
}

int patient_malloc(size_t bytes, void **out, int attempts = 4)
{
    hipError_t e = hipSuccess;
    for (int attempt = 0; attempt < attempts; ++attempt) {
        e = hipMalloc(out, bytes);
        if (e == hipSuccess) return TOMO_OK;
        (void)hipGetLastError();
        if (e != hipErrorOutOfMemory || attempt + 1 == attempts) break;
        struct timespec ts = {0, 300 * 1000 * 1000};
        nanosleep(&ts, nullptr);
    }
    *out = nullptr;
    return tomo_fail(e == hipErrorOutOfMemory ? TOMO_E_NOMEM : TOMO_E_RUNTIME, "hipMalloc of %zu bytes of scratch failed: %s", bytes,
                     hipGetErrorString(e));
}

int placed_malloc(hipStream_t st, size_t bytes, void **out)
{
    std::lock_guard<std::mutex> lk(g_place_mu);
    const int tries = placement_tries();
    if (bytes < PLACE_MIN_BYTES || tries <= 1) return patient_malloc(bytes, out);
    size_t free0 = 0, total = 0;
    if (hipMemGetInfo(&free0, &total) != hipSuccess) { (void)hipGetLastError(); return patient_malloc(bytes, out); }
    const size_t hold_cap = (size_t)(PLACE_HOLD_FRACTION * (double)free0);
    void *cand[PLACE_MAX_TRIES];
    place_rec rec;
    rec.bytes = bytes;
    double lo = 0.0;
    for (int t = 0; t < tries; ++t) {
        if (t > 0) {
            size_t fr = 0, tot = 0;
            if ((size_t)(t + 1) * bytes > hold_cap) break;
            if (hipMemGetInfo(&fr, &tot) != hipSuccess || fr < bytes + PLACE_HEADROOM) { (void)hipGetLastError(); break; }
        }
        void *p = nullptr;
        if (t == 0) {
            const int rc = patient_malloc(bytes, &p);
            if (rc != TOMO_OK) return rc;
        } else if (hipMalloc(&p, bytes) != hipSuccess) {
            (void)hipGetLastError();
            break;
        }
        cand[t] = p;
        rec.score[t] = place_score(p, bytes, st);
        rec.tries = t + 1;
        if (rec.chosen < 0 || rec.score[t] > rec.score[rec.chosen]) rec.chosen = t;
        lo = (t == 0) ? rec.score[t] : std::min(lo, rec.score[t]);
        if (t >= 1 && lo > 0.0 && rec.score[rec.chosen] >= PLACE_FAST_GAIN * lo) { rec.fast = 1; break; }
    }
    for (int t = 0; t < rec.tries; ++t)
        if (t != rec.chosen) (void)hipFree(cand[t]);
    *out = cand[rec.chosen];
    g_place_last = rec;
    return TOMO_OK;
}
}

extern "C" int tomo_set_placement_tries(int tries)
{
    TOMO_REQUIRE(tries >= 1 && tries <= PLACE_MAX_TRIES, "placement tries must be 1 .. %d", PLACE_MAX_TRIES);
    std::lock_guard<std::mutex> lk(g_place_mu);
    g_place_tries = tries;
    return TOMO_OK;
}

extern "C" int tomo_placement_tries(void)
{
    std::lock_guard<std::mutex> lk(g_place_mu);
    return placement_tries();
}

extern "C" int tomo_placement_last(size_t *bytes, int *chosen, double *scores_GBps, int capacity)
{
    std::lock_guard<std::mutex> lk(g_place_mu);
    if (bytes) *bytes = g_place_last.bytes;
    if (chosen) *chosen = g_place_last.chosen;
    for (int t = 0; scores_GBps && t < capacity && t < g_place_last.tries; ++t) scores_GBps[t] = g_place_last.score[t];
    return g_place_last.tries;
}

extern "C" int tomo_placement_last_fast(void)
{
    std::lock_guard<std::mutex> lk(g_place_mu);
    return g_place_last.tries > 0 ? g_place_last.fast : -1;
}

int tomo_arena_get(int device, hipStream_t stream, int slot, size_t bytes, void **out, bool place)
{
    void *old = nullptr;
    {
        std::lock_guard<std::mutex> lk(g_arena_mu);
        arena_t &a = g_arenas[arena_key{device, stream, slot}];
        if (a.bytes >= bytes) { *out = a.ptr; return TOMO_OK; }
        old = a.ptr;
        a.ptr = nullptr;
        a.bytes = 0;
    }
    if (old) {
        const hipError_t es = hipStreamSynchronize(stream);
        const hipError_t ef = hipFree(old);
        TOMO_HIP(es);
        TOMO_HIP(ef);
    }
    void *p = nullptr;
    const int rc = place ? placed_malloc(stream, bytes, &p) : patient_malloc(bytes, &p, slot == ARENA_BPQ ? 1 : 4);
    if (rc != TOMO_OK) return rc;
    std::lock_guard<std::mutex> lk(g_arena_mu);
    arena_t &a = g_arenas[arena_key{device, stream, slot}];
    if (a.ptr != nullptr) {
        (void)hipFree(p);
        return tomo_fail(TOMO_E_INVALID, "two host threads grew the scratch arena of one (device, stream, slot) at the same time");
    }
    a.ptr = p;
    a.bytes = bytes;
    *out = p;
    return TOMO_OK;
}

extern "C" int tomo_reserve_scratch(int device, size_t bytes, void *stream)
{
    TOMO_REQUIRE(device >= 0 && bytes > 0, "bad scratch reservation");
    TOMO_ON_DEVICE(device);
    void *p = nullptr;
    return tomo_arena_get(device, as_stream(stream), ARENA_TV, bytes, &p, true);
}

extern "C" int tomo_placed_scratch(int device, int slot, size_t bytes, void *stream, void **out_dev)
{
    TOMO_REQUIRE(device >= 0 && slot >= 0 && slot < 8 && bytes > 0 && out_dev != nullptr, "bad placed-scratch request (slot 0 .. 7)");
    TOMO_ON_DEVICE(device);
    return tomo_arena_get(device, as_stream(stream), ARENA_CALLER0 + slot, bytes, out_dev, true);
}

int tomo_arena_release_slot(int device, int slot)
{
    std::lock_guard<std::mutex> lk(g_arena_mu);
    bool any = false;
    for (auto it = g_arenas.begin(); it != g_arenas.end();) {
        if (it->first.device == device && it->first.slot == slot && it->second.ptr) {
            tomo_device_guard g(device);
            if (!any) { TOMO_HIP(hipDeviceSynchronize()); any = true; }
            TOMO_HIP(hipFree(it->second.ptr));
            it = g_arenas.erase(it);
        } else {
            ++it;
        }
    }
    return TOMO_OK;
}

extern "C" int tomo_release_scratch(int device)
{
    tomo_fourier_cache_release(device);
    tomo_fbp_cache_release(device);
    tomo_bp_relay_reset(device);
    std::lock_guard<std::mutex> lk(g_arena_mu);
    bool any = false;
    for (auto it = g_arenas.begin(); it != g_arenas.end();) {
        if (it->first.device == device && it->second.ptr) {
            if (!any) {
                TOMO_ON_DEVICE(device);
                TOMO_HIP(hipDeviceSynchronize());
                any = true;
            }
            tomo_device_guard g(device);
            TOMO_HIP(hipFree(it->second.ptr));
            it = g_arenas.erase(it);
        } else {
            ++it;
        }
    }
    return TOMO_OK;
}

struct prof_rec { hipEvent_t a, b; long long launches; };
static std::mutex g_prof_mu;
static bool g_prof_on = false;
static std::vector<prof_rec> g_prof[PROF_CLASSES];

tomo_prof_scope::tomo_prof_scope(int cls_, hipStream_t st_, int launches_) : cls(cls_), st(st_), launches(launches_), rec(nullptr)
{
    if (!g_prof_on) return;
    prof_rec *r = new prof_rec();
    r->launches = launches;
    if (hipEventCreate(&r->a) != hipSuccess || hipEventCreate(&r->b) != hipSuccess) { delete r; return; }
    (void)hipEventRecord(r->a, st);
    rec = r;
}

tomo_prof_scope::~tomo_prof_scope()
{
    if (!rec) return;
    prof_rec *r = (prof_rec *)rec;
    (void)hipEventRecord(r->b, st);
    std::lock_guard<std::mutex> lk(g_prof_mu);
    g_prof[cls].push_back(*r);
    delete r;
}

static void prof_clear()
{
    for (auto &v : g_prof) {
        for (auto &r : v) { (void)hipEventDestroy(r.a); (void)hipEventDestroy(r.b); }
        v.clear();
    }
}

extern "C" int tomo_profile_enable(int on)
{
    std::lock_guard<std::mutex> lk(g_prof_mu);
    prof_clear();
    g_prof_on = on != 0;
    return TOMO_OK;
}

extern "C" int tomo_profile_read(const char *kernel, long long *launches, double *total_ms)
{
    TOMO_REQUIRE(kernel && launches && total_ms, "NULL argument");
    std::string k(kernel);
    int cls = k == "bp" ? PROF_BP : k == "fp" ? PROF_FP : k == "pdtv" ? PROF_PDTV : k == "roftv" ? PROF_ROFTV : -1;
    TOMO_REQUIRE(cls >= 0, "unknown kernel '%s'", kernel);
    std::lock_guard<std::mutex> lk(g_prof_mu);
    long long n = 0;
    double ms = 0.0;
    for (auto &r : g_prof[cls]) {
        TOMO_HIP(hipEventSynchronize(r.b));
        float t = 0.0f;
        TOMO_HIP(hipEventElapsedTime(&t, r.a, r.b));
        ms += t;
        n += r.launches;
    }
    *launches = n;
    *total_ms = ms;
    return TOMO_OK;
}
```

tomobar_amd/csrc/tomo_common.h:

```cpp
#pragma once
#include <hip/hip_runtime.h>
#include <hip/hip_fp16.h>

#include <cstdarg>
#include <cstdint>
#include <cstdio>
#include <string>
#include <vector>

#include "tomo_mi355x.h"

int tomo_fail(int code, const char *fmt, ...);

#define TOMO_HIP(expr)                                                                          \
    do {                                                                                        \
        hipError_t e_ = (expr);                                                                 \
        if (e_ != hipSuccess)                                                                   \
            return tomo_fail(e_ == hipErrorOutOfMemory ? TOMO_E_NOMEM : TOMO_E_RUNTIME,          \
                             "%s failed: %s (%s:%d)", #expr, hipGetErrorString(e_), __FILE__,   \
                             __LINE__);                                                         \
    } while (0)

#define TOMO_LAUNCH_CHECK()                                                                     \
    do {                                                                                        \
        hipError_t e_ = hipGetLastError();                                                      \
        if (e_ != hipSuccess)                                                                   \
            return tomo_fail(TOMO_E_RUNTIME, "kernel launch failed: %s (%s:%d)",                \
                             hipGetErrorString(e_), __FILE__, __LINE__);                        \
    } while (0)

#define TOMO_REQUIRE(cond, ...)                                                                 \
    do {                                                                                        \
        if (!(cond)) return tomo_fail(TOMO_E_INVALID, __VA_ARGS__);                              \
    } while (0)

struct tomo_subset {
    int size = 0;
    size_t table_offset = 0;
    int n_dirx = 0;
    int n_class[4] = {0, 0, 0, 0};
    int wbound[4] = {0, 0, 0, 0};
    int wbound_wide[4] = {0, 0, 0, 0};
    int wbound16[4] = {0, 0, 0, 0};
};

struct tomo_ctx {
    int device = 0;
    int nz = 0, n = 0, nu = 0, na = 0;
    int os = 1, bins = 0;
    unsigned flags = 0;
    std::vector<int64_t> newind;
    std::vector<tomo_angle_t> host_table;
    std::vector<tomo_subset> subsets;
    tomo_angle_t *dev_table = nullptr;
    std::vector<int> host_fp_order;
    int *dev_fp_order = nullptr;
    int *dev_fp_mult = nullptr;
    void *scratch = nullptr;
    size_t scratch_bytes = 0;
    const float *volT_of = nullptr;
    bool volT_valid = false;
    hipStream_t volT_stream = nullptr;
    std::string last_fp_path, last_bp_path;
    int res_layout = 0;
};

void tomo_warn_once(const char *key, const char *msg);

struct tomo_device_guard {
    int prev = -1;
    hipError_t err = hipSuccess;
    explicit tomo_device_guard(int device)
    {
        err = hipGetDevice(&prev);
        if (err == hipSuccess && prev != device) err = hipSetDevice(device);
        else if (err == hipSuccess) prev = -1;
    }
    ~tomo_device_guard() { if (prev >= 0) (void)hipSetDevice(prev); }
    tomo_device_guard(const tomo_device_guard &) = delete;
    tomo_device_guard &operator=(const tomo_device_guard &) = delete;
};
#define TOMO_ON_DEVICE(dev)                 \
    tomo_device_guard device_guard_(dev);   \
    TOMO_HIP(device_guard_.err)

static inline hipStream_t as_stream(void *s) { return reinterpret_cast<hipStream_t>(s); }

enum { ARENA_MAIN = 0, ARENA_REDUCE = 1, ARENA_TV = 2 , ARENA_BPQ = 3 , ARENA_TVSNAP = 4 , ARENA_CALLER0 = 16  };
int tomo_arena_get(int device, hipStream_t stream, int slot, size_t bytes, void **out, bool place = false);
int tomo_arena_release_slot(int device, int slot);
int fp_tables(tomo_ctx *ctx);
void tomo_bp_relay_reset(int device);
void tomo_fourier_cache_release(int device);
void tomo_fbp_cache_release(int device);

extern thread_local int g_variant_bp, g_variant_fp, g_variant_pdtv, g_variant_roftv;
#ifdef TOMO_DEV_VARIANTS
#define TOMO_DEV 1
extern thread_local int g_probe;
#else
#define TOMO_DEV 0
constexpr int g_probe = 0;
#endif

static inline int ceil_div(int a, int b) { return (a + b - 1) / b; }

enum { PROF_BP = 0, PROF_FP = 1, PROF_PDTV = 2, PROF_ROFTV = 3, PROF_CLASSES = 4 };
struct tomo_prof_scope {
    int cls;
    hipStream_t st;
    int launches;
    void *rec;
    tomo_prof_scope(int cls, hipStream_t st, int launches);
    ~tomo_prof_scope();
};
```

tomobar_amd/methodsIR_CuPy.py:

```python

from __future__ import annotations

from typing import Optional, Union

import numpy as np
import torch
from numpy import float32

from . import ops
from .convergence import check_tolerance, relative_change
from .projector import HipTools3D, geom_size
from .regularisersCuPy import check_prox_available, last_prox, prox_regul, reserve_prox_scratch
from .supp.dicts import dicts_check
from .supp.regularisers import has_wavelets
from .supp.suppTools import _apply_horiz_detector_padding, check_kwargs, perform_recon_crop


class _RunMonitor:

    def __init__(self, rt, method: str, a: dict, start, r: Optional[dict] = None):
        self.slab = rt.slab
        self.tol = check_tolerance(a.get("tolerance"), "_algorithm_['tolerance']")
        self.inner = (r is not None and r.get("method") is not None
                      and check_tolerance(r.get("tolerance"), "_regularisation_['tolerance']") > 0.0)
        self.verbose = bool(a.get("verbose"))
        self.snap = start.clone() if self.tol > 0.0 else None
        self.run = rt.last_run = {"method": method, "iterations_done": int(a["iterations"]), "converged": False,
                                  "rel_change": [], "prox_iterations": []}

    def prox_done(self) -> None:
        if self.inner:
            self.run["prox_iterations"].append(last_prox()[0])

    def stop(self, k: int, v) -> bool:
        if self.snap is None:
            return False
        pair = ops.rel_change(v, self.snap, self.snap)
        if self.slab is not None:
            pair = self.slab.allreduce_sums(pair)
        d = relative_change(*pair)
        self.run["rel_change"].append(d)
        if not d < self.tol:
            return False
        self.run["iterations_done"], self.run["converged"] = k, True
        if self.verbose:
            print(f"{self.run['method']} stopped after iteration {k}: relative change {d:.3e} < tolerance {self.tol:.3e}")
        return True


class RecToolsIRCuPy:

    def __init__(self, DetectorsDimH: int, DetectorsDimH_pad: int, DetectorsDimV: Union[int, None],
                 CenterRotOffset: Union[float, np.ndarray], AnglesVec: np.ndarray, ObjSize: int,
                 device_projector: int = 0, OS_number: Optional[int] = None, adjoint: str = "unmatched"):
        self.OS_number = OS_number
        self.objsize_user_given = ObjSize if DetectorsDimH_pad != 0 else None
        if DetectorsDimH_pad > 0:
            ObjSize = DetectorsDimH + 2 * DetectorsDimH_pad
        if DetectorsDimV == 0 or DetectorsDimV is None:
            DetectorsDimV = 1
        self.geom = "3D"
        self.Atools = HipTools3D(DetectorsDimH, DetectorsDimH_pad, DetectorsDimV, AnglesVec, CenterRotOffset,
                                 ObjSize, "gpu", device_projector, OS_number,
                                 **({} if adjoint == "unmatched" else {"adjoint": adjoint}))
        self.power_seed = None
        self.last_run = None
        self.slab = None

    @property
    def slab(self):
        return self._slab

    @slab.setter
    def slab(self, comm):
        self._slab = comm
        self.Atools.slab = comm

    @property
    def adjoint(self) -> str:
        return self.Atools.adjoint

    @adjoint.setter
    def adjoint(self, value):
        self.Atools.adjoint = value

    @property
    def OS_number(self) -> int:
        return self._OS_number

    @OS_number.setter
    def OS_number(self, value):
        self._OS_number = 1 if value is None else value

    @property
    def objsize_user_given(self):
        return self._objsize_user_given

    @objsize_user_given.setter
    def objsize_user_given(self, value):
        self._objsize_user_given = value

    def reserve_scratch(self, _regularisation_: Union[dict, None]) -> None:
        if _regularisation_ is not None and _regularisation_.get("method") is not None:
            reserve_prox_scratch(self, self.Atools.vol_shape(), _regularisation_)

    def _Ax(self, x, sub_ind: int = 1, os: bool = False):
        return self.Atools._forwprojOSCuPy(x, os_index=sub_ind) if os else self.Atools._forwprojCuPy(x)

    def _Atb(self, b, sub_ind: int = 1, os: bool = False):
        return self.Atools._backprojOSCuPy(b, os_index=sub_ind) if os else self.Atools._backprojCuPy(b)

    def _gdot(self, x, y) -> float:
        v = ops.dot(x, y)
        return v if self.slab is None else self.slab.allreduce_sum(v)

    def _new_vol(self, fill=None):
        v = torch.empty(self.Atools.vol_shape(), dtype=torch.float32, device=self.Atools._device)
        if fill is not None:
            ops.fill(v, fill)
        return v

    def _prepare_data(self, _data_, _algorithm_, _regularisation_, method_run):
        self._given = _data_.get("projection_data") if isinstance(_data_, dict) else None
        d, a, r = dicts_check(self, _data_, _algorithm_, _regularisation_, method_run=method_run)
        check_prox_available(self, self.Atools.vol_shape(), r)
        d["projection_data"] = _apply_horiz_detector_padding(d["projection_data"], self.Atools.detectors_x_pad, True)
        expect = self.Atools.sino_shape(None)
        if tuple(d["projection_data"].shape) != expect:
            raise ValueError(f"projection data has shape {tuple(d['projection_data'].shape)} after axis swap and "
                             f"padding, the geometry expects {expect}")
        if d["projection_data"].dtype != torch.float32:
            raise ValueError("projection data must be float32")
        return d, a, r

    def _finalise(self, x, _algorithm_):
        given = getattr(self, "_given", None)
        self._given = None
        if self.objsize_user_given is not None:
            return ops.like(perform_recon_crop(x, self.objsize_user_given), given)
        return ops.like(check_kwargs(x, cupyrun=True, recon_mask_radius=_algorithm_["recon_mask_radius"]), given)

    def __common_initialisation(self, _data_, _algorithm_, _regularisation_, method_run):
        d, a, r = self._prepare_data(_data_, _algorithm_, _regularisation_, method_run)
        if a.get("lipschitz_const") is None:
            a["lipschitz_const"] = self.powermethod(d)
        rec_dim = geom_size(self.Atools.vol_geom)
        x0 = None
        if a["initialise"] is not None:
            if tuple(a["initialise"].shape) == rec_dim:
                x0 = ops.contiguous(ops.to_device(a["initialise"], self.Atools.device_index)).clone()
            else:
                print(f"Provided initialisation (array) has incorrect dimensions, the correct dims are {rec_dim}. "
                      "Zero initialisation is used.")
        if x0 is None:
            x0 = self._new_vol(1.0 if method_run == "OSEM" else 0.0)
        use_os = self.OS_number > 1
        w = ops.pwls_weights(d["projection_data"], self.slab) if _data_["data_fidelity"] in ["PWLS", "SWLS"] else None
        reserve_prox_scratch(self, rec_dim, r)
        return (d, a, r, x0, w, use_os)

    def powermethod(self, _data_: dict) -> float:
        if _data_.get("data_fidelity") is None:
            _data_["data_fidelity"] = "LS"
        A = self.Atools
        gen = None
        if self.power_seed is not None:
            gen = torch.Generator(device=A._device)
            gen.manual_seed(int(self.power_seed))
        x1 = torch.randn(A.vol_shape(), dtype=torch.float32, device=A._device, generator=gen)
        sub = 0 if self.OS_number > 1 else None
        y = A.forward(x1, sub)
        s = 1.0
        for _ in range(15):
            A.backward(y, sub, out=x1)
            s = ops.norm2(x1)
            if self.slab is not None:
                s = float(np.sqrt(self.slab.allreduce_sum(s * s)))
            s = float32(s)
            ops.scale(float32(1.0) / s, x1, x1)
            A.forward(x1, sub, out=y)
        return float(s)

    def FISTA(self, _data_: dict, _algorithm_: Union[dict, None] = None,
              _regularisation_: Union[dict, None] = None) -> torch.Tensor:
        (d, a, r, x0, w, use_os) = self.__common_initialisation(_data_, _algorithm_, _regularisation_, "FISTA")
        A = self.Atools
        L_inv = float32(1.0 / a["lipschitz_const"])
        b = d["projection_data"]
        fid = self.data_fidelity
        nonneg = bool(a["nonnegativity"])
        has_prox = r["method"] is not None

        ring_lambda = d.get("ringGH_lambda")
        use_ring = ring_lambda is not None
        use_swls = fid == "SWLS"
        robust = None
        if d.get("huber_threshold") is not None:
            robust = ("huber", float32(d["huber_threshold"]))
        elif d.get("studentst_threshold") is not None:
            robust = ("studentst", float32(d["studentst_threshold"]))
        if use_ring:
            ring_acc = float32(d["ringGH_accelerate"])
            r_shape = (A.nz, A.nu)
            r_cur = torch.zeros(r_shape, dtype=torch.float32, device=A._device)
            r_old = torch.zeros(r_shape, dtype=torch.float32, device=A._device)
            r_x = torch.zeros(r_shape, dtype=torch.float32, device=A._device)

        t = float32(1.0)
        X = x0
        X_t = x0.clone()
        res = {}
        X_grad = self._new_vol() if has_prox else None
        X_prox = self._new_vol() if has_prox else None

        A.invalidate()
        zquad = not (use_ring or use_swls) and not getattr(A, "has_vertical_shift", False)
        A.set_residual_layout("zquad" if zquad else "planar")
        n_sub_total = a["iterations"] * self.OS_number
        mon = _RunMonitor(self, "FISTA", a, x0, r)
        try:
            for it_no in range(a["iterations"]):
                for sub_ind in range(self.OS_number):
                    sub = sub_ind if use_os else None
                    t_old = t
                    if sub not in res:
                        res[sub] = A.residual_buffer(sub)
                    if use_ring:
                        A.residual_ring(X_t, b, r_x, ring_acc, sub, res[sub])
                        A.ring_reduce(res[sub], w if fid == "PWLS" else None, r_x, L_inv, sub, r_cur)
                        if robust is not None:
                            A.robust_apply(res[sub], *robust)
                    elif use_swls:
                        A.residual(X_t, b, None, "LS", sub, res[sub])
                        A.swls_apply(res[sub], w, float32(d["beta_SWLS"]), sub)
                        if robust is not None:
                            A.robust_apply(res[sub], *robust)
                    else:
                        A.residual(X_t, b, w, fid, sub, res[sub], robust=robust)
                    t = float32((float32(1.0) + np.sqrt(float32(1.0) + float32(4.0) * t * t)) * float32(0.5))
                    beta = float32((t_old - float32(1.0)) / t)
                    if not has_prox:
                        A.grad_step_momentum(res[sub], X_t, X, L_inv, beta, nonneg, sub)
                    else:
                        A.grad_step(res[sub], X_t, X_grad, L_inv, nonneg, sub)
                        prox_regul(self, X_grad, r, out=X_prox)
                        mon.prox_done()
                        if it_no * self.OS_number + sub_ind + 1 < n_sub_total:
                            A.momentum(X_prox, X, X_t, beta)
                        X, X_prox = X_prox, X
                    if use_ring:
                        A.ring_update(r_cur, r_old, r_x, float32(ring_lambda), beta)
                if mon.stop(it_no + 1, X):
                    break
        finally:
            A.set_residual_layout("planar")
            A.invalidate()
        return self._finalise(X, a)

    def ADMM(self, _data_: dict, _algorithm_: Union[dict, None] = None,
             _regularisation_: Union[dict, None] = None) -> torch.Tensor:
        (d, a, r, x0, w, use_os) = self.__common_initialisation(_data_, _algorithm_, _regularisation_, "ADMM")
        A = self.Atools
        b = d["projection_data"]
        fid = self.data_fidelity
        nonneg = bool(a["nonnegativity"])
        has_prox = r["method"] is not None
        rho, alpha = a["ADMM_rho_const"], a["ADMM_relax_par"]
        tau = float32(0.9 / (a["lipschitz_const"] + rho))
        r_local = dict(r)
        if has_prox:
            r_local["regul_param"] = r["regul_param"] / rho
            if ("LLT_ROF" in r["method"] or has_wavelets(r["method"])) and "regul_param2" in r:
                r_local["regul_param2"] = r["regul_param2"] / rho

        x = x0
        z = x0.clone()
        u = self._new_vol(0.0)
        zu = self._new_vol()
        res = {}
        A.set_residual_layout("planar" if getattr(A, "has_vertical_shift", False) else "zquad")
        mon = _RunMonitor(self, "ADMM", a, x0, r)
        try:
            for iter_no in range(a["iterations"]):
                for sub_ind in range(self.OS_number):
                    sub = sub_ind if use_os else None
                    if sub not in res:
                        res[sub] = A.residual_buffer(sub)
                    A.residual(z, b, w, fid, sub, res[sub])
                    A.admm_z_update(res[sub], z, x, u, zu, tau, float32(rho), iter_no > 1, float32(1.0 - alpha),
                                    float32(alpha), nonneg, sub)
                    if has_prox:
                        prox_regul(self, zu, r_local, out=x)
                        mon.prox_done()
                    else:
                        x, zu = zu, x
                ops.admm_dual(u, z, x)
                if a["verbose"] and np.mod(iter_no, (round)(a["iterations"] / 5) + 1) == 0:
                    print("ADMM iteration (", iter_no + 1, ") using", r["method"], "regularisation")
                if mon.stop(iter_no + 1, x):
                    break
        finally:
            A.set_residual_layout("planar")
        return self._finalise(x, a)

    def Landweber(self, _data_: dict, _algorithm_: Union[dict, None] = None) -> torch.Tensor:
        d, a, _ = self._prepare_data(_data_, _algorithm_, None, "Landweber")
        A = self.Atools
        b = d["projection_data"]
        x = self._new_vol(0.0)
        step = float32(a["tau_step_lanweber"])
        A.set_residual_layout("planar" if getattr(A, "has_vertical_shift", False) else "zquad")
        try:
            res = A.residual_buffer(None)
            mon = _RunMonitor(self, "Landweber", a, x)
            for k in range(a["iterations"]):
                A.residual(x, b, None, "LS", None, res)
                A.grad_step(res, x, x, step, a["nonnegativity"], None)
                if mon.stop(k + 1, x):
                    break
        finally:
            A.set_residual_layout("planar")
        return self._finalise(x, a)

    def SIRT(self, _data_: dict, _algorithm_: Union[dict, None] = None) -> torch.Tensor:
        d, a, _ = self._prepare_data(_data_, _algorithm_, None, "SIRT")
        A = self.Atools
        b = d["projection_data"]
        ones_v = self._new_vol(1.0)
        R = A.forward(ones_v)
        ops.recip_safe(R, R)
        ones_s = torch.empty_like(b)
        ops.fill(ones_s, 1.0)
        Cm = A.backward(ones_s)
        ops.recip_safe(Cm, Cm)
        del ones_s
        x = ones_v
        res = torch.empty_like(b)
        upd = self._new_vol()
        mon = _RunMonitor(self, "SIRT", a, x)
        for k in range(a["iterations"]):
            A.forward(x, None, out=res)
            ops.axpby(1.0, b, -1.0, res)
            ops.mul(R, res)
            A.backward(res, None, out=upd)
            ops.mul(Cm, upd)
            ops.axpby(1.0, upd, 1.0, x)
            if a["nonnegativity"]:
                ops.clamp_min(x, 0.0)
            if mon.stop(k + 1, x):
                break
        return self._finalise(x, a)

    def CGLS(self, _data_: dict, _algorithm_: Union[dict, None] = None) -> torch.Tensor:
        d, a, _ = self._prepare_data(_data_, _algorithm_, None, "CGLS")
        A = self.Atools
        x = self._new_vol(0.0)
        r_vec = d["projection_data"].clone()
        dvec = A.backward(r_vec)
        normr2 = float32(self._gdot(dvec, dvec))
        Ad = torch.empty_like(r_vec)
        s = self._new_vol()
        mon = _RunMonitor(self, "CGLS", a, x)
        for k in range(a["iterations"]):
            A.forward(dvec, None, out=Ad)
            alpha = float32(normr2 / float32(self._gdot(Ad, Ad)))
            ops.axpby(alpha, dvec, 1.0, x)
            ops.axpby(-alpha, Ad, 1.0, r_vec)
            A.backward(r_vec, None, out=s)
            normr2_new = float32(self._gdot(s, s))
            beta = float32(normr2_new / normr2)
            normr2 = normr2_new
            ops.axpby(1.0, s, beta, dvec)
            if a["nonnegativity"]:
                ops.clamp_min(x, 0.0)
            if mon.stop(k + 1, x):
                break
        return self._finalise(x, a)

    def OSEM(self, _data_: dict, _algorithm_: Union[dict, None] = None,
             _regularisation_: Union[dict, None] = None) -> torch.Tensor:
        (d, a, r, x, w, use_os) = self.__common_initialisation(_data_, _algorithm_, _regularisation_, "OSEM")
        A = self.Atools
        b = d["projection_data"]
        eps = 1e-8
        sub0 = 0 if use_os else None
        ones_s = torch.empty(A.sino_shape(sub0), dtype=torch.float32, device=A._device)
        ops.fill(ones_s, 1.0)
        normalisation = A.backward(ones_s, sub0)
        ops.clamp_min(normalisation, eps)
        del ones_s
        ratio, back = {}, self._new_vol()
        mon = _RunMonitor(self, "OSEM", a, x, r)
        for k in range(a["iterations"]):
            for sub_ind in range(self.OS_number):
                sub = sub_ind if use_os else None
                if sub not in ratio:
                    ratio[sub] = torch.empty(A.sino_shape(sub), dtype=torch.float32, device=A._device)
                A.residual(x, b, None, "RATIO", sub, ratio[sub])
                A.backward(ratio[sub], sub, out=back)
                ops.mul(normalisation, back)
                ops.mul(back, x)
                if r["method"] is not None:
                    x = prox_regul(self, x, r)
                    mon.prox_done()
            if mon.stop(k + 1, x):
                break
        return self._finalise(x, a)
```

tomobar_amd/projector.py:

```python

from __future__ import annotations

import ctypes as C
from typing import Optional, Union

import numpy as np
import torch

from . import _lib as L
from . import ops


def geom_size(geom: dict) -> tuple:
    if "GridRowCount" in geom:
        return (geom["GridSliceCount"], geom["GridRowCount"], geom["GridColCount"])
    return (geom["DetectorRowCount"], geom["Vectors"].shape[0], geom["DetectorColCount"])


def vec_geom_init3D(angles_rad, DetectorSpacingX, DetectorSpacingY, CenterRotOffset) -> np.ndarray:
    th = np.asarray(angles_rad, dtype=np.float64).ravel()
    c, s = np.cos(th), np.sin(th)
    cor = np.asarray(CenterRotOffset, dtype=np.float64)
    if cor.ndim == 0:
        c0, c1 = np.full_like(th, float(cor)), np.zeros_like(th)
    elif cor.ndim == 1:
        c0, c1 = cor, np.zeros_like(th)
    else:
        c0, c1 = cor[:, 0], cor[:, 1]
    out = np.zeros((th.size, 12))
    out[:, 0], out[:, 1] = s, -c
    out[:, 3], out[:, 4], out[:, 5] = c * c0, s * c0, c1
    out[:, 6], out[:, 7] = c * DetectorSpacingX, s * DetectorSpacingX
    out[:, 11] = DetectorSpacingY
    return out


class HipTools3D:

    def __init__(self, detectors_x: int, detectors_x_pad: int, detectors_y: int, angles_vec: np.ndarray,
                 centre_of_rotation: Union[float, np.ndarray], recon_size: int, processing_arch: str = "gpu",
                 device_index: int = 0, ordsub_number: Optional[int] = None, lerp8: bool = False,
                 adjoint: str = "unmatched"):
        if detectors_x <= 0:
            raise ValueError("The size of the horizontal detector cannot be negative or zero")
        if detectors_x_pad < 0:
            raise ValueError("The padding size of the horizontal detector cannot be negative")
        if len(angles_vec) == 0:
            raise ValueError("The length of angles array cannot be zero")
        if np.ndim(angles_vec) >= 2:
            raise ValueError("The array of angles must be 1D")
        if np.ndim(centre_of_rotation) == 1 and len(centre_of_rotation) != len(angles_vec):
            raise ValueError("The CoR must be a scalar or a 1D array of the SAME size as angles")
        if centre_of_rotation is None:
            centre_of_rotation = 0.0
        if isinstance(recon_size, tuple):
            raise ValueError("Reconstruction is currently available for squared or cubic objects only, please provide a scalar")
        if recon_size <= 0:
            raise ValueError("The size of the reconstruction object cannot be zero")
        if processing_arch not in ("cpu", "gpu"):
            raise ValueError("Please choose the processing architecture to be either 'cpu' or 'gpu'")
        if processing_arch == "cpu":
            raise ValueError("3D CPU reconstruction is not supported, please use GPU")
        if device_index <= -2:
            raise ValueError("The GPU device index can be only -1, 0 and larger than 0")
        if ordsub_number is None:
            ordsub_number = 1
        if ordsub_number <= 0:
            raise ValueError("The number of ordered subsets cannot be negative or zero")
        if detectors_y is not None and detectors_y <= 0:
            raise ValueError("The size of the vertical detector cannot be negative or zero")
        self.lerp8 = bool(lerp8)
        self._adjoint = self._check_adjoint(adjoint)

        self.detectors_x = int(detectors_x)
        self.detectors_x_pad = int(detectors_x_pad)
        self.detectors_y = int(detectors_y)
        self.angles_vec = np.ascontiguousarray(angles_vec, dtype=np.float64)
        self.centre_of_rotation = centre_of_rotation
        self.recon_size = int(recon_size)
        self.processing_arch = processing_arch
        self.device_index = int(device_index)
        self.ordsub_number = int(ordsub_number)

        self.nz, self.n = self.detectors_y, self.recon_size
        self._vshift = None
        self.slab = None
        self.nu = self.detectors_x + 2 * self.detectors_x_pad
        self.na = self.angles_vec.size

        cor = np.asarray(centre_of_rotation, dtype=np.float64)
        if cor.ndim == 0:
            cor_arr, stride = cor.reshape(1).copy(), 0
        elif cor.ndim == 1:
            cor_arr, stride = np.ascontiguousarray(cor), 1
        elif cor.ndim == 2 and cor.shape == (self.na, 2):
            cor_arr, stride = np.ascontiguousarray(cor[:, 0]), 1
            if np.any(cor[:, 1] != 0):
                self._vshift = np.ascontiguousarray(cor[:, 1], dtype=np.float32)
        else:
            raise ValueError("The CoR must be a scalar, a vector [angles] or an array [angles, 2]")

        self._device = ops._require_gpu(self.device_index)
        self._lib = L.lib()
        handle = C.c_void_p()
        self._chk(self._lib.tomo_ctx_create(
            self.device_index, self.nz, self.n, self.nu, self.na,
            self.angles_vec.ctypes.data_as(C.POINTER(C.c_double)), cor_arr.ctypes.data_as(C.POINTER(C.c_double)),
            stride, self.ordsub_number, L.FLAG_LERP8 if lerp8 else 0, C.byref(handle)))
        self._ctx = handle

        self.vol_geom = {"GridRowCount": self.n, "GridColCount": self.n, "GridSliceCount": self.nz,
                         "option": {"WindowMinX": -self.n / 2, "WindowMaxX": self.n / 2,
                                    "WindowMinY": -self.n / 2, "WindowMaxY": self.n / 2,
                                    "WindowMinZ": -self.nz / 2, "WindowMaxZ": self.nz / 2}}
        self.NumbProjBins = self._lib.tomo_ctx_num_bins(self._ctx)
        table = np.zeros((self.ordsub_number, self.NumbProjBins), dtype=np.int64)
        self._chk(self._lib.tomo_ctx_newind_table(self._ctx, table.ctypes.data_as(C.POINTER(C.c_int64))))
        self.newInd_Vec = table
        if self.ordsub_number == 1:
            self.proj_geom = self._proj_geom(np.arange(self.na))
        else:
            self.proj_geom_OS = {s: self._proj_geom(self.subset_indices(s)) for s in range(self.ordsub_number)}

    def _proj_geom(self, idx):
        cor = self.centre_of_rotation
        cor_sel = cor if np.ndim(cor) == 0 else np.asarray(cor)[idx]
        return {"type": "parallel3d_vec", "DetectorRowCount": self.nz, "DetectorColCount": self.nu,
                "Vectors": vec_geom_init3D(self.angles_vec[idx], 1.0, 1.0, cor_sel)}

    def subset_indices(self, sub_ind: int) -> np.ndarray:
        ind = self.newInd_Vec[sub_ind, :]
        if ind[self.NumbProjBins - 1] == 0:
            ind = ind[:-1]
        return ind

    def subset_size(self, os_index) -> int:
        return self._lib.tomo_ctx_subset_size(self._ctx, -1 if os_index is None else int(os_index))

    def vol_shape(self):
        return (self.nz, self.n, self.n)

    def sino_shape(self, os_index=None):
        return (self.nz, self.subset_size(os_index), self.nu)

    def _sub(self, os_index):
        return -1 if (os_index is None or self.ordsub_number == 1) else int(os_index)

    def _vol_in(self, x):
        x = ops.contiguous(ops.to_device(x, self.device_index))
        ops._chk_f32(x, "volume")
        if tuple(x.shape) != self.vol_shape():
            raise ValueError(f"volume has shape {tuple(x.shape)}, expected {self.vol_shape()}")
        return x

    def _sino_in(self, b, os_index):
        b = ops.contiguous(ops.to_device(b, self.device_index))
        ops._chk_f32(b, "projection data")
        if tuple(b.shape) != self.sino_shape(os_index):
            raise ValueError(f"projection data has shape {tuple(b.shape)}, expected {self.sino_shape(os_index)}")
        return b

    def _check_adjoint(self, value):
        if value not in ("unmatched", "matched"):
            raise ValueError(f"adjoint should be 'unmatched' or 'matched', not {value!r}")
        if value == "matched" and self.lerp8:
            raise ValueError("adjoint='matched' is the transpose of the unquantised forward projector: "
                             "it is not available with lerp8=True")
        return value

    @property
    def adjoint(self) -> str:
        return self._adjoint

    @adjoint.setter
    def adjoint(self, value):
        self._adjoint = self._check_adjoint(value)
        if value == "matched" and self.residual_layout() != "planar":
            self.set_residual_layout("planar")

    def _bp_name(self, name, adjoint=None):
        matched = self._check_adjoint(adjoint or self._adjoint) == "matched"
        return getattr(self._lib, name.replace("tomo_bp3d", "tomo_bp3d_matched") if matched else name)

    def _forwprojCuPy(self, object3D):
        return self.forward(object3D, None)

    def _forwprojOSCuPy(self, object3D, os_index: int):
        return self.forward(object3D, os_index)

    def _backprojCuPy(self, proj_data):
        return self.backward(proj_data, None)

    def _backprojOSCuPy(self, proj_data, os_index: int):
        return self.backward(proj_data, os_index)

    @property
    def has_vertical_shift(self) -> bool:
        return self._vshift is not None

    def _shift_rows(self, sino, os_index, sign, out=None):
        key = self._sub(os_index)
        tabs = self.__dict__.setdefault("_vshift_tables", {})
        if key not in tabs:
            idx = np.arange(self.na) if key < 0 else self.subset_indices(key)
            tabs[key] = torch.from_numpy(np.ascontiguousarray(self._vshift[idx])).to(self._device)
        if out is None:
            out = torch.empty_like(sino)
        slab = self.slab
        if slab is not None and slab.world > 1:
            from .slab import check_ghost_rows, extend_detector_rows
            g = int(np.ceil(float(np.abs(self._vshift).max()))) + 1
            if getattr(self, "_vshift_checked", None) is not slab:
                check_ghost_rows(slab, g, self.nz, f"a vertical CoR component of up to {float(np.abs(self._vshift).max()):.2f} rows")
                self._vshift_checked = slab
            ext, lo = extend_detector_rows(slab, sino, g)
            ext_out = torch.empty_like(ext)
            with torch.cuda.device(self._device):
                self._chk(self._lib.tomo_shift_rows(ops.ptr(ext), ops.ptr(ext_out), int(ext.shape[0]), int(sino.shape[1]), self.nu,
                                                ops.ptr(tabs[key]), float(sign), ops.stream_ptr(sino)))
            out.copy_(ext_out[lo:lo + self.nz])
            return out
        with torch.cuda.device(self._device):
            self._chk(self._lib.tomo_shift_rows(ops.ptr(sino), ops.ptr(out), self.nz, int(sino.shape[1]), self.nu,
                                            ops.ptr(tabs[key]), float(sign), ops.stream_ptr(sino)))
        return out

    def _adjoint_in(self, res, os_index):
        return res if self._vshift is None else self._shift_rows(res, os_index, -1.0)

    def forward(self, vol, os_index=None, out=None):
        vol = self._vol_in(vol)
        if out is None:
            out = torch.empty(self.sino_shape(os_index), dtype=torch.float32, device=self._device)
        if self._vshift is not None:
            tmp = torch.empty_like(out)
            with torch.cuda.device(self._device):
                self._chk(self._lib.tomo_fp3d(self._ctx, self._sub(os_index), ops.ptr(vol), ops.ptr(tmp), ops.stream_ptr(vol)))
            return self._shift_rows(tmp, os_index, 1.0, out)
        with torch.cuda.device(self._device):
            self._chk(self._lib.tomo_fp3d(self._ctx, self._sub(os_index), ops.ptr(vol), ops.ptr(out), ops.stream_ptr(vol)))
        return out

    def backward(self, sino, os_index=None, out=None, adjoint=None):
        sino = self._adjoint_in(self._sino_in(sino, os_index), os_index)
        if out is None:
            out = torch.empty(self.vol_shape(), dtype=torch.float32, device=self._device)
        with torch.cuda.device(self._device):
            self._chk(self._bp_name("tomo_bp3d", adjoint)(self._ctx, self._sub(os_index), ops.ptr(sino), ops.ptr(out), ops.stream_ptr(sino)))
        return out

    def set_residual_layout(self, layout: str):
        if layout == "zquad" and self._adjoint == "matched":
            layout = "planar"
        if layout == "zquad" and self._vshift is not None:
            raise ValueError("the quad-interleaved residual is not available with a vertical CoR component")
        self._chk(self._lib.tomo_ctx_set_residual_layout(self._ctx, L.RESIDUAL_LAYOUT[layout]))

    def residual_layout(self) -> str:
        code = self._lib.tomo_ctx_residual_layout(self._ctx)
        return {v: k for k, v in L.RESIDUAL_LAYOUT.items()}[code]

    def residual_buffer(self, os_index=None) -> torch.Tensor:
        if self.residual_layout() == "planar":
            return torch.empty(self.sino_shape(os_index), dtype=torch.float32, device=self._device)
        n = int(self._lib.tomo_ctx_residual_elems(self._ctx, self._sub(os_index)))
        return torch.empty((n // (4 * self.nu * self.subset_size(os_index)), self.subset_size(os_index), self.nu, 4),
                           dtype=torch.float32, device=self._device)

    def _check_residual(self, res, os_index):
        want = int(self._lib.tomo_ctx_residual_elems(self._ctx, self._sub(os_index)))
        quad = self.residual_layout() == "zquad"
        if res.numel() != want or (res.dim() == 4) != quad:
            raise ValueError(f"residual buffer of {res.numel()} floats / rank {res.dim()} does not match the context's current "
                             f"'{self.residual_layout()}' layout ({want} floats): take it from residual_buffer() after "
                             "set_residual_layout(), and do not share one projector object between drivers running concurrently")

    def residual_as_planar(self, res, os_index=None) -> torch.Tensor:
        if res.dim() == 3:
            return res
        return res.permute(0, 3, 1, 2).reshape(-1, res.shape[1], res.shape[2])[: self.nz].contiguous()

    def residual(self, vol, b, w, fidelity: str, os_index, out, gathered: int = 0, robust=None):
        if self._vshift is None:
            self._check_residual(out, os_index)
        if robust is not None:
            mode, delta = robust
            if self._vshift is not None:
                self.residual(vol, b, w, fidelity, os_index, out, gathered)
                return self.robust_apply(out, mode, delta)
            with torch.cuda.device(self._device):
                self._chk(self._lib.tomo_fp3d_residual_robust(self._ctx, self._sub(os_index), ops.ptr(vol), ops.ptr(b),
                                                          ops.ptr(w), int(gathered), L.FID[fidelity], L.ROBUST[mode],
                                                          float(delta), ops.ptr(out), ops.stream_ptr(vol)))
            return out
        if self._vshift is not None:
            ax = self.forward(vol, os_index)
            src = self._src_table(os_index)
            with torch.cuda.device(self._device):
                self._chk(self._lib.tomo_sino_residual(ops.ptr(ax), ops.ptr(b), ops.ptr(w), ops.ptr(src), self.nz,
                                                   int(src.numel()), self.na, self.nu, int(gathered), L.FID[fidelity],
                                                   ops.ptr(out),
                                                   ops.stream_ptr(vol)))
            return out
        with torch.cuda.device(self._device):
            self._chk(self._lib.tomo_fp3d_residual(self._ctx, self._sub(os_index), ops.ptr(vol), ops.ptr(b),
                                               ops.ptr(w), int(gathered), L.FID[fidelity], ops.ptr(out),
                                               ops.stream_ptr(vol)))
        return out

    def _src_table(self, os_index):
        key = self._sub(os_index)
        tabs = self.__dict__.setdefault("_src_tables", {})
        if key not in tabs:
            idx = np.arange(self.na) if key < 0 else self.subset_indices(key)
            tabs[key] = torch.from_numpy(np.ascontiguousarray(idx, dtype=np.int32)).to(self._device)
        return tabs[key]

    def residual_ring(self, vol, b, r_x, accelerate, os_index, out):
        if self._vshift is not None:
            self.residual(vol, b, None, "LS", os_index, out)
            with torch.cuda.device(self._device):
                self._chk(self._lib.tomo_sino_add_ring(ops.ptr(out), ops.ptr(r_x), float(accelerate), self.nz,
                                                   self.subset_size(os_index), self.nu, ops.stream_ptr(vol)))
            return out
        with torch.cuda.device(self._device):
            self._chk(self._lib.tomo_fp3d_residual_ring(self._ctx, self._sub(os_index), ops.ptr(vol), ops.ptr(b), ops.ptr(r_x),
                                                    float(accelerate), ops.ptr(out), ops.stream_ptr(vol)))
        return out

    def ring_reduce(self, res, w, r_x, l_inv, os_index, r_out):
        src = self._src_table(os_index)
        with torch.cuda.device(self._device):
            self._chk(self._lib.tomo_ring_gh_reduce(ops.ptr(res), ops.ptr(w), ops.ptr(src), self.nz, int(src.numel()), self.na,
                                                self.nu, ops.ptr(r_x), float(l_inv), ops.ptr(r_out), ops.stream_ptr(res)))

    def swls_apply(self, res, w, beta, os_index):
        src = self._src_table(os_index)
        with torch.cuda.device(self._device):
            self._chk(self._lib.tomo_swls_apply(ops.ptr(res), ops.ptr(w), ops.ptr(src), self.nz, int(src.numel()), self.na,
                                            self.nu, float(beta), ops.stream_ptr(res)))

    def robust_apply(self, res, mode: str, delta):
        with torch.cuda.device(self._device):
            self._chk(self._lib.tomo_sino_robust(ops.ptr(res), res.numel(), L.ROBUST[mode], float(delta), ops.stream_ptr(res)))
        return res

    def ring_update(self, r, r_old, r_x, lam, beta):
        with torch.cuda.device(self._device):
            self._chk(self._lib.tomo_ring_gh_update(ops.ptr(r), ops.ptr(r_old), ops.ptr(r_x), float(lam), float(beta),
                                                r.numel(), ops.stream_ptr(r)))

    def momentum(self, x, x_old, x_t, beta):
        with torch.cuda.device(self._device):
            self._chk(self._lib.tomo_momentum_transposed(self._ctx, ops.ptr(x), ops.ptr(x_old), ops.ptr(x_t), float(beta),
                                                     ops.stream_ptr(x)))

    def invalidate(self):
        self._chk(self._lib.tomo_ctx_invalidate(self._ctx))

    def grad_step(self, res, x_t, x_out, l_inv, nonneg, os_index):
        if self._vshift is None:
            self._check_residual(res, os_index)
        res = self._adjoint_in(res, os_index)
        with torch.cuda.device(self._device):
            self._chk(self._bp_name("tomo_bp3d_fista")(self._ctx, self._sub(os_index), ops.ptr(res), ops.ptr(x_t), ops.ptr(x_out),
                                            float(l_inv), int(bool(nonneg)), ops.stream_ptr(x_t)))

    def grad_step_momentum(self, res, x_t, x_old_then_x, l_inv, beta, nonneg, os_index):
        if self._vshift is None:
            self._check_residual(res, os_index)
        res = self._adjoint_in(res, os_index)
        with torch.cuda.device(self._device):
            self._chk(self._bp_name("tomo_bp3d_fista_momentum")(self._ctx, self._sub(os_index), ops.ptr(res), ops.ptr(x_t),
                                                     ops.ptr(x_old_then_x), float(l_inv), float(beta),
                                                     int(bool(nonneg)), ops.stream_ptr(x_t)))

    def admm_z_update(self, res, z, x, u, zu_out, tau, rho, relax_on, one_minus_alpha, alpha, nonneg, os_index):
        if self._vshift is None:
            self._check_residual(res, os_index)
        res = self._adjoint_in(res, os_index)
        with torch.cuda.device(self._device):
            self._chk(self._bp_name("tomo_bp3d_admm")(self._ctx, self._sub(os_index), ops.ptr(res), ops.ptr(z), ops.ptr(x),
                                           ops.ptr(u), ops.ptr(zu_out), float(tau), float(rho), int(bool(relax_on)),
                                           float(one_minus_alpha), float(alpha), int(bool(nonneg)), ops.stream_ptr(z)))

    def angle_table(self, os_index=None):
        n = self.subset_size(os_index)
        tab = (L.AngleRecord * max(n, 1))()
        self._chk(self._lib.tomo_ctx_angle_table(self._ctx, self._sub(os_index), tab, max(n, 1)))
        return tab, n

    def kernel_path(self, op: str = "fp") -> str:
        return self._lib.tomo_ctx_kernel_path(self._ctx, op.encode()).decode()

    def _chk(self, rc):
        L.check(rc, self._lib)

    def release_scratch(self):
        self._chk(self._lib.tomo_ctx_release_scratch(self._ctx))

    def __del__(self):
        ctx = getattr(self, "_ctx", None)
        if ctx:
            try:
                self._lib.tomo_ctx_destroy(ctx)
            except Exception:
                pass
            self._ctx = None


AstraTools3D = HipTools3D
```

Before: 0.7264 iterations/s.

## Store FISTA momentum volume quad-interleaved in z for forward and back projection

Adds a z-quad interleaved volume layout (four slices packed per float4) that the momentum kernel writes together with a transposed copy, so the forward projector can read it with vector loads and LDS-DMA staging. The back-projection FISTA epilogue also reads it. A 13-angle grouping variant is added for whole-row forward launches when it does not increase padding. The FISTA driver enables this when a prox is used and every subset qualifies. It adds layout plumbing, a transpose kernel and alignment requirements, and other solver paths are restricted to the planar layout.

```diff
diff --git a/include/tomo_mi355x.h b/include/tomo_mi355x.h
--- a/include/tomo_mi355x.h
+++ b/include/tomo_mi355x.h
@@ -100,6 +100,13 @@
 int tomo_ctx_set_residual_layout(tomo_ctx *ctx, int layout);
 int tomo_ctx_residual_layout(const tomo_ctx *ctx);
 size_t tomo_ctx_residual_elems(const tomo_ctx *ctx, int subset);
+
+enum { TOMO_VOLUME_PLANAR = 0, TOMO_VOLUME_ZQUAD = 1 };
+int tomo_ctx_set_volume_layout(tomo_ctx *ctx, int layout);
+int tomo_ctx_volume_layout(const tomo_ctx *ctx);
+size_t tomo_ctx_volume_elems(const tomo_ctx *ctx);
+int tomo_ctx_volume_zquad_ok(const tomo_ctx *ctx, int subset);
+int tomo_volume_to_zquad(tomo_ctx *ctx, const float *x_dev, float *xq_dev, void *stream);
 
 int tomo_momentum(const float *x_dev, const float *xold_dev, float *xt_dev, float beta, size_t count, void *stream);
 int tomo_momentum_transposed(tomo_ctx *ctx, const float *x_dev, const float *xold_dev, float *xt_dev, float beta,
diff --git a/tomobar_amd/_lib.py b/tomobar_amd/_lib.py
--- a/tomobar_amd/_lib.py
+++ b/tomobar_amd/_lib.py
@@ -15,6 +15,7 @@
 FID = {"LS": 0, "PWLS": 1, "KL": 2, "RATIO": 3}
 ROBUST = {None: 0, "huber": 1, "studentst": 2}
 RESIDUAL_LAYOUT = {"planar": 0, "zquad": 1}
+VOLUME_LAYOUT = {"planar": 0, "zquad": 1}
 NDF_PENALTY = {"Huber": 0, "PM": 1, "Tukey": 2}
 
 
@@ -67,6 +68,11 @@
     "tomo_ctx_set_residual_layout": (_i, [_vp, _i]),
     "tomo_ctx_residual_layout": (_i, [_vp]),
     "tomo_ctx_residual_elems": (_sz, [_vp, _i]),
+    "tomo_ctx_set_volume_layout": (_i, [_vp, _i]),
+    "tomo_ctx_volume_layout": (_i, [_vp]),
+    "tomo_ctx_volume_elems": (_sz, [_vp]),
+    "tomo_ctx_volume_zquad_ok": (_i, [_vp, _i]),
+    "tomo_volume_to_zquad": (_i, [_vp, _vp, _vp, _vp]),
     "tomo_momentum": (_i, [_vp, _vp, _vp, _f, _sz, _vp]),
     "tomo_momentum_transposed": (_i, [_vp, _vp, _vp, _vp, _f, _vp]),
     "tomo_ctx_invalidate": (_i, [_vp]),
diff --git a/tomobar_amd/csrc/proj_kernels.hip b/tomobar_amd/csrc/proj_kernels.hip
--- a/tomobar_amd/csrc/proj_kernels.hip
+++ b/tomobar_amd/csrc/proj_kernels.hip
@@ -39,6 +39,7 @@
     int nz, n, nu, na;
     float *vol;
     const float *xt;
+    int xt_zquad;
     float *xout;
     float *xt_out;
     const float *xold;
@@ -315,6 +316,12 @@
         a.epi_aligned = (bits & 15) == 0;
     }
     if (EPI == EPI_PLAIN) a.zquad = 0;
+    if (EPI != EPI_FISTA) a.xt_zquad = 0;
+    if (a.xt_zquad) {
+        TOMO_REQUIRE((((uintptr_t)a.xt) & 15) == 0, "the quad-interleaved volume must be 16-byte aligned");
+        TOMO_REQUIRE((g_variant_bp == 0 || g_variant_bp == 3) && (long)a.na * a.nu < (1L << 25),
+                     "this back projection does not read the quad-interleaved volume");
+    }
     if (a.zquad && (((uintptr_t)a.sino) & 15) != 0)
         return tomo_fail(TOMO_E_INVALID, "the quad-interleaved residual must be 16-byte aligned");
     bool relaid = false;
@@ -513,6 +520,62 @@
     }
 }
 
+template <bool MOMENTUM>
+__global__ __launch_bounds__(256) void zquad64_kernel(const float *__restrict__ x, const float *__restrict__ xold,
+                                                      float *__restrict__ xq, float *__restrict__ xq_T, float beta, int n, int nz)
+{
+    __shared__ float t[4][64][64];
+    const size_t plane = (size_t)n * n;
+    const int z0 = 4 * (int)blockIdx.z;
+    const int bx = blockIdx.x * 64, by = blockIdx.y * 64;
+    const int c4 = (threadIdx.x & 15) * 4, r0 = threadIdx.x >> 4;
+    float4 av[4][4], ov[4][4];
+#pragma unroll
+    for (int k = 0; k < 4; ++k)
+#pragma unroll
+        for (int zz = 0; zz < 4; ++zz) {
+            const int xx = bx + c4, yy = by + r0 + 16 * k;
+            av[k][zz] = ov[k][zz] = make_float4(0.0f, 0.0f, 0.0f, 0.0f);
+            if (xx < n && yy < n && z0 + zz < nz) {
+                const size_t i = (size_t)(z0 + zz) * plane + (size_t)yy * n + xx;
+                av[k][zz] = nt_ld4(x + i);
+                if (MOMENTUM) ov[k][zz] = nt_ld4(xold + i);
+            }
+        }
+#pragma unroll
+    for (int k = 0; k < 4; ++k) {
+        const int r = r0 + 16 * k;
+#pragma unroll
+        for (int zz = 0; zz < 4; ++zz) {
+            const float4 a = av[k][zz], o = ov[k][zz];
+            float4 v = a;
+            if (MOMENTUM) {
+                v.x = a.x + beta * (a.x - o.x); v.y = a.y + beta * (a.y - o.y);
+                v.z = a.z + beta * (a.z - o.z); v.w = a.w + beta * (a.w - o.w);
+            }
+            t[zz][r][(c4 + r) & 63] = v.x; t[zz][r][(c4 + 1 + r) & 63] = v.y;
+            t[zz][r][(c4 + 2 + r) & 63] = v.z; t[zz][r][(c4 + 3 + r) & 63] = v.w;
+        }
+    }
+    __syncthreads();
+    const int lane = threadIdx.x & 63, w = threadIdx.x >> 6;
+    const size_t qoff = (size_t)blockIdx.z * plane;
+#pragma unroll 4
+    for (int m = 0; m < 16; ++m) {
+        const int r = w + 4 * m;
+        const int s = (lane + r) & 63;
+        if (bx + lane < n && by + r < n)
+            nt_st4(xq + 4 * (qoff + (size_t)(by + r) * n + bx + lane), make_float4(t[0][r][s], t[1][r][s], t[2][r][s], t[3][r][s]));
+    }
+#pragma unroll 4
+    for (int m = 0; m < 16; ++m) {
+        const int r = w + 4 * m;
+        const int s = (r + lane) & 63;
+        if (bx + r < n && by + lane < n)
+            nt_st4(xq_T + 4 * (qoff + (size_t)(bx + r) * n + by + lane), make_float4(t[0][lane][s], t[1][lane][s], t[2][lane][s], t[3][lane][s]));
+    }
+}
+
 static inline bool aligned16(const void *a, const void *b, const void *c, const void *d)
 {
 #ifdef TOMO_GLUE32
@@ -680,10 +743,13 @@
     size_t lds;
     long blocks;
     bool mult;
+    bool qv;
+    int group;
 };
 
 struct FpPlan {
     bool march = false;
+    bool qv = false;
     int count = 0;
     FpLaunch l[4];
 };
@@ -746,7 +812,26 @@
     return {FP_TILED, cls, false, off, nc, wp, 256, passes, kc, nut, ngroups, lds, blocks, false};
 }
 
-static int fp_plan(const tomo_ctx *ctx, const tomo_subset &s, int variant, FpPlan &plan)
+constexpr int FP_A13 = 13;
+static bool fp_plan_group13(const tomo_ctx *ctx, const tomo_subset &s, FpLaunch &l)
+{
+    if (ceil_div(l.n_angles, FP_A13) * FP_A13 > ceil_div(l.n_angles, FP_A) * FP_A) return false;
+    const int wp = s.wbound_wide13[l.cls], passes = ceil_div(wp, l.threads);
+    if (wp <= 0 || passes > 2) return false;
+    const size_t tab = (size_t)ctx->n * 8;
+    int kc = 4;
+    size_t lds = (size_t)2 * kc * wp * 16 + tab;
+    if (lds > 160 * 1024) { kc = 2; lds = (size_t)2 * kc * wp * 16 + tab; }
+    if (lds > 160 * 1024) return false;
+    l.wpitch = wp; l.passes = passes; l.kc = kc; l.lds = lds;
+    l.ngroups = ceil_div(l.n_angles, FP_A13);
+    l.blocks = fp_blocks(ctx->nz, l.nut, l.ngroups);
+    l.mult = l.mult && (size_t)2 * l.threads * 16 <= lds - tab;
+    l.group = FP_A13;
+    return true;
+}
+
+static int fp_plan(const tomo_ctx *ctx, const tomo_subset &s, int variant, FpPlan &plan, bool volq = false)
 {
     constexpr double FP_DENSE16_PAYS = 0.75;
     plan = FpPlan();
@@ -804,6 +889,12 @@
         TOMO_REQUIRE(plan.l[i].form != FP_TILED_SYNC || plan.l[i].lds <= 64 * 1024,
                      "forward-projection window does not fit in LDS");
     }
+    if (volq && ctx->n % 4 == 0) {
+        plan.qv = plan.count > 0;
+        for (int i = 0; i < plan.count; ++i) plan.qv &= plan.l[i].form == FP_WHOLE_ROW && plan.l[i].passes <= 2;
+        for (int i = 0; i < plan.count; ++i) plan.l[i].qv = plan.qv;
+        for (int i = 0; i < plan.count && plan.qv; ++i) (void)fp_plan_group13(ctx, s, plan.l[i]);
+    }
     return TOMO_OK;
 }
 
@@ -813,7 +904,9 @@
     switch (l.form) {
     case FP_WHOLE_ROW:
         return std::string(l.cls >> 1 ? "x" : "y") + (l.merged ? "" : (l.cls & 1) ? "-" : "+") + ":whole-row(" +
-               std::to_string(l.threads) + " threads, " + passes + ", " + std::to_string(l.kc) + " rows/chunk) ";
+               std::to_string(l.threads) + " threads, " + passes + ", " + std::to_string(l.kc) + " rows/chunk" +
+               (l.qv ? ", quad-interleaved volume, LDS-DMA staging" + std::string(l.group ? ", " + std::to_string(l.group) + " angles) " : ") ")
+                     : ") ");
     case FP_DENSE16: return cls + "dense(256 pixels x 16 angles, " + passes + ") ";
     case FP_TILED: return cls + "tiled-pipelined(256 threads, " + passes + ") ";
     default: return cls + "tiled-sync(window " + std::to_string(l.wpitch) + ") ";
@@ -831,7 +924,13 @@
         fp_tiled_sync_kernel<L8, RES, 256, FP_A><<<(unsigned)l.blocks, 256, l.lds, st>>>(t, l.kc);
         return;
     case FP_WHOLE_ROW:
-        if (l.passes == 1) k = fp_tiled_kernel<L8, RES, 1, 4, true, 1024>;
+        if (l.qv && l.group == FP_A13 && l.passes == 1) k = fp_tiled_kernel<L8, RES, 1, 4, true, 1024, FP_A13, true>;
+        else if (l.qv && l.group == FP_A13 && m == 8) k = fp_tiled_kernel<L8, RES, 2, 8, true, 1024, FP_A13, true>;
+        else if (l.qv && l.group == FP_A13) k = fp_tiled_kernel<L8, RES, 2, 4, true, 1024, FP_A13, true>;
+        else if (l.qv && l.passes == 1) k = fp_tiled_kernel<L8, RES, 1, 4, true, 1024, FP_A, true>;
+        else if (l.qv && m == 8) k = fp_tiled_kernel<L8, RES, 2, 8, true, 1024, FP_A, true>;
+        else if (l.qv) k = fp_tiled_kernel<L8, RES, 2, 4, true, 1024, FP_A, true>;
+        else if (l.passes == 1) k = fp_tiled_kernel<L8, RES, 1, 4, true, 1024>;
         else if (l.passes == 2 && m == 8) k = fp_tiled_kernel<L8, RES, 2, 8, true, 1024>;
         else if (l.passes == 2) k = fp_tiled_kernel<L8, RES, 2, 4, true, 1024>;
         else if (l.passes == 3 && m == 6) k = fp_tiled_kernel<L8, RES, 3, 6, false, 1024>;
@@ -856,22 +955,29 @@
 
 int fp_run(tomo_ctx *ctx, int subset, const float *vol, const float *b, const float *w, int gathered, int fidelity,
            float *out, void *stream, const float *ring = nullptr, float ring_scale = 0.0f, int zquad = 0,
-           int robust = TOMO_ROBUST_NONE, float rdelta = 0.0f)
+           int robust = TOMO_ROBUST_NONE, float rdelta = 0.0f, int volq = 0)
 {
     TOMO_REQUIRE(ctx != nullptr, "ctx is NULL");
     TOMO_REQUIRE(vol != nullptr && out != nullptr, "NULL data pointer");
     TOMO_REQUIRE(subset < ctx->os, "subset %d out of range (OS_number %d)", subset, ctx->os);
     const tomo_subset &s = (subset < 0 || ctx->os == 1) ? ctx->subsets[0] : ctx->subsets[1 + subset];
     hipStream_t st = as_stream(stream);
-    const bool ready = ctx->volT_valid && ctx->volT_of == vol && ctx->volT_stream == st && ctx->scratch != nullptr;
+    const bool ready = ctx->volT_valid && ctx->volT_of == vol && ctx->volT_stream == st && ctx->scratch != nullptr &&
+                       ctx->volT_quad == (volq != 0);
     ctx->volT_valid = false;
     ctx->volT_of = nullptr;
     if (s.size == 0) return TOMO_OK;
     TOMO_ON_DEVICE(ctx->device);
+    const int variant = g_variant_fp == 5 ? 0 : g_variant_fp;
     FpArgs a;
     a.vol = vol;
     a.volT = nullptr;
-    if (s.n_dirx > 0) {
+    if (volq) {
+        TOMO_REQUIRE((((uintptr_t)vol) & 15) == 0, "the quad-interleaved volume must be 16-byte aligned");
+        TOMO_REQUIRE(s.n_dirx == 0 || ready, "a quad-interleaved volume is forward projected once, right after tomo_momentum_transposed / "
+                                             "tomo_volume_to_zquad wrote it on the same stream");
+        a.volT = (const float *)ctx->scratch;
+    } else if (s.n_dirx > 0) {
         int rc = fp_scratch(ctx);
         if (rc != TOMO_OK) return rc;
         if (!ready) {
@@ -898,11 +1004,13 @@
     ctx->last_fp_path.clear();
     const bool l8 = (ctx->flags & TOMO_FLAG_LERP8) != 0;
     FpPlan plan;
-    const int rc = fp_plan(ctx, s, g_variant_fp, plan);
+    const int rc = fp_plan(ctx, s, variant, plan, volq != 0);
     if (rc != TOMO_OK) return rc;
+    TOMO_REQUIRE(!volq || plan.qv, "this subset's forward projection does not read the quad-interleaved volume "
+                                   "(tomo_ctx_volume_zquad_ok says so beforehand)");
     if (plan.march) {
         ctx->last_fp_path = "march(no LDS)";
-        if (g_variant_fp != 1) tomo_warn_once("fp_march", "forward projection: a staged row window exceeds 64 KiB of LDS, "
+        if (variant != 1) tomo_warn_once("fp_march", "forward projection: a staged row window exceeds 64 KiB of LDS, "
                                               "falling back to the un-tiled march kernel (about 4x slower)");
         dim3 grid(ceil_div(ctx->nu, 256), s.size, ceil_div(ctx->nz, 4));
         if (b) {
@@ -969,8 +1077,10 @@
                 s.wbound[c] = fp_window_bound(tab, order + o, nc, n, nu);
                 s.wbound16[c] = fp_window_bound(tab, order + o, nc, n, nu, 256, FP_A16);
                 if (nu > 1024) s.wbound_wide[c] = fp_window_bound(tab, order + o, nc, n, nu, bt);
+                if (nu > 1024) s.wbound_wide13[c] = fp_window_bound(tab, order + o, nc, n, nu, bt, FP_A13);
             }
             if (nu <= 1024 && nc0 + nc1 > 0) s.wbound_wide[2 * d] = fp_window_bound(tab, order + off, nc0 + nc1, n, nu, bt);
+            if (nu <= 1024 && nc0 + nc1 > 0) s.wbound_wide13[2 * d] = fp_window_bound(tab, order + off, nc0 + nc1, n, nu, bt, FP_A13);
             off += nc0 + nc1;
         }
     }
@@ -1007,7 +1117,8 @@
                  "data_fidelity should be LS, PWLS or KL");
     TOMO_REQUIRE(fidelity != TOMO_FID_PWLS || w_full_dev != nullptr, "PWLS needs the weights");
     return fp_run(ctx, subset, vol_dev, b_full_dev, fidelity == TOMO_FID_PWLS ? w_full_dev : nullptr, gathered,
-                  fidelity, res_dev, stream, nullptr, 0.0f, ctx ? ctx->res_layout : 0);
+                  fidelity, res_dev, stream, nullptr, 0.0f, ctx ? ctx->res_layout : 0, TOMO_ROBUST_NONE, 0.0f,
+                  ctx ? ctx->vol_layout : 0);
 }
 
 extern "C" int tomo_fp3d_residual_robust(tomo_ctx *ctx, int subset, const float *vol_dev, const float *b_full_dev,
@@ -1020,7 +1131,7 @@
     TOMO_REQUIRE(robust == TOMO_ROBUST_NONE || robust == TOMO_ROBUST_HUBER || robust == TOMO_ROBUST_STUDENTST, "unknown robust mode %d", robust);
     TOMO_REQUIRE(robust == TOMO_ROBUST_NONE || delta > 0.0f, "the Huber / Student's-t threshold must be positive");
     return fp_run(ctx, subset, vol_dev, b_full_dev, fidelity == TOMO_FID_PWLS ? w_full_dev : nullptr, gathered,
-                  fidelity, res_dev, stream, nullptr, 0.0f, ctx ? ctx->res_layout : 0, robust, delta);
+                  fidelity, res_dev, stream, nullptr, 0.0f, ctx ? ctx->res_layout : 0, robust, delta, ctx ? ctx->vol_layout : 0);
 }
 
 extern "C" int tomo_ctx_set_residual_layout(tomo_ctx *ctx, int layout)
@@ -1041,10 +1152,80 @@
     return nzr * (size_t)s.size * (size_t)ctx->nu;
 }
 
+extern "C" int tomo_ctx_set_volume_layout(tomo_ctx *ctx, int layout)
+{
+    TOMO_REQUIRE(ctx != nullptr, "ctx is NULL");
+    TOMO_REQUIRE(layout == TOMO_VOLUME_PLANAR || layout == TOMO_VOLUME_ZQUAD, "unknown volume layout %d", layout);
+    TOMO_REQUIRE(layout == TOMO_VOLUME_PLANAR || ctx->n % 4 == 0, "the quad-interleaved volume needs a slice size that is a multiple of 4");
+    ctx->vol_layout = layout;
+    ctx->volT_valid = false;
+    ctx->volT_of = nullptr;
+    return TOMO_OK;
+}
+
+extern "C" int tomo_ctx_volume_layout(const tomo_ctx *ctx) { return ctx ? ctx->vol_layout : -1; }
+
+extern "C" size_t tomo_ctx_volume_elems(const tomo_ctx *ctx)
+{
+    if (!ctx) return 0;
+    const size_t nzv = ctx->vol_layout == TOMO_VOLUME_ZQUAD ? (size_t)ceil_div(ctx->nz, 4) * 4 : (size_t)ctx->nz;
+    return nzv * (size_t)ctx->n * (size_t)ctx->n;
+}
+
+extern "C" int tomo_ctx_volume_zquad_ok(const tomo_ctx *ctx, int subset)
+{
+    if (!ctx || subset >= ctx->os || ctx->n % 4 != 0 || ceil_div(ctx->nz, 4) > 65535) return 0;
+    if (g_variant_fp != 0 || (g_variant_bp != 0 && g_variant_bp != 3)) return 0;
+    const tomo_subset &s = (subset < 0 || ctx->os == 1) ? ctx->subsets[0] : ctx->subsets[1 + subset];
+    if (s.size == 0 || (long)s.size * ctx->nu >= (1L << 25)) return 0;
+    FpPlan plan;
+    if (fp_plan(ctx, s, 0, plan, true) != TOMO_OK) return 0;
+    return plan.qv ? 1 : 0;
+}
+
+static int fp_scratch_zquad(tomo_ctx *ctx)
+{
+    const size_t need = (size_t)ceil_div(ctx->nz, 4) * 4 * ctx->n * ctx->n * sizeof(float);
+    if (ctx->scratch_bytes < need) {
+        ctx->volT_valid = false;
+        if (ctx->scratch) { TOMO_HIP(hipDeviceSynchronize()); TOMO_HIP(hipFree(ctx->scratch)); ctx->scratch = nullptr; ctx->scratch_bytes = 0; }
+        TOMO_HIP(hipMalloc(&ctx->scratch, need));
+        ctx->scratch_bytes = need;
+    }
+    return TOMO_OK;
+}
+
+static int volume_zquad_produce(tomo_ctx *ctx, const float *x_dev, const float *xold_dev, float *xq_dev, float beta, void *stream)
+{
+    TOMO_REQUIRE(ctx->n % 4 == 0 && aligned16(x_dev, xold_dev, xq_dev, nullptr),
+                 "the quad-interleaved volume needs a slice size that is a multiple of 4 and 16-byte aligned arrays");
+    const int nq = ceil_div(ctx->nz, 4);
+    TOMO_REQUIRE(nq <= 65535, "too many slices for one launch");
+    TOMO_ON_DEVICE(ctx->device);
+    int rc = fp_scratch_zquad(ctx);
+    if (rc != TOMO_OK) return rc;
+    dim3 tg(ceil_div(ctx->n, 64), ceil_div(ctx->n, 64), nq);
+    if (xold_dev) zquad64_kernel<true><<<tg, 256, 0, as_stream(stream)>>>(x_dev, xold_dev, xq_dev, (float *)ctx->scratch, beta, ctx->n, ctx->nz);
+    else zquad64_kernel<false><<<tg, 256, 0, as_stream(stream)>>>(x_dev, nullptr, xq_dev, (float *)ctx->scratch, 0.0f, ctx->n, ctx->nz);
+    TOMO_LAUNCH_CHECK();
+    ctx->volT_of = xq_dev;
+    ctx->volT_stream = as_stream(stream);
+    ctx->volT_quad = true;
+    ctx->volT_valid = true;
+    return TOMO_OK;
+}
+
+extern "C" int tomo_volume_to_zquad(tomo_ctx *ctx, const float *x_dev, float *xq_dev, void *stream)
+{
+    TOMO_REQUIRE(ctx != nullptr && x_dev && xq_dev, "NULL argument");
+    return volume_zquad_produce(ctx, x_dev, nullptr, xq_dev, 0.0f, stream);
+}
+
 extern "C" int tomo_momentum_transposed(tomo_ctx *ctx, const float *x_dev, const float *xold_dev, float *xt_dev, float beta,
                                         void *stream)
 {
     TOMO_REQUIRE(ctx != nullptr && x_dev && xold_dev && xt_dev, "NULL argument");
+    if (ctx->vol_layout == TOMO_VOLUME_ZQUAD) return volume_zquad_produce(ctx, x_dev, xold_dev, xt_dev, beta, stream);
     TOMO_ON_DEVICE(ctx->device);
     int rc = fp_scratch(ctx);
     if (rc != TOMO_OK) return rc;
@@ -1058,6 +1239,7 @@
     TOMO_LAUNCH_CHECK();
     ctx->volT_of = xt_dev;
     ctx->volT_stream = as_stream(stream);
+    ctx->volT_quad = false;
     ctx->volT_valid = true;
     return TOMO_OK;
 }
@@ -1076,6 +1258,7 @@
     TOMO_REQUIRE(b_full_dev != nullptr && ring_dev != nullptr, "projection data / ring offset pointer is NULL");
     TOMO_REQUIRE(ctx == nullptr || ctx->res_layout == TOMO_RESIDUAL_PLANAR,
                  "the ring-term residual is read by tomo_ring_gh_reduce in the planar layout: set TOMO_RESIDUAL_PLANAR first");
+    TOMO_REQUIRE(ctx == nullptr || ctx->vol_layout == TOMO_VOLUME_PLANAR, "the ring-term residual takes the planar volume: set TOMO_VOLUME_PLANAR first");
     return fp_run(ctx, subset, vol_dev, b_full_dev, nullptr, 0, TOMO_FID_LS, res_dev, stream, ring_dev, ring_scale);
 }
 
@@ -1098,6 +1281,7 @@
     TOMO_REQUIRE(xt_dev && xout_dev, "NULL volume pointer");
     a.xt = xt_dev; a.xout = xout_dev; a.s0 = l_inv; a.nonneg = nonneg;
     a.zquad = ctx->res_layout == TOMO_RESIDUAL_ZQUAD;
+    a.xt_zquad = ctx->vol_layout == TOMO_VOLUME_ZQUAD;
     return bp_launch<EPI_FISTA>(a, (ctx->flags & TOMO_FLAG_LERP8) != 0, as_stream(stream));
 }
 
@@ -1108,6 +1292,7 @@
     int rc = bp_prepare(ctx, subset, res_dev, a);
     if (rc != TOMO_OK) return rc;
     TOMO_REQUIRE(xt_dev && xold_x_dev, "NULL volume pointer");
+    TOMO_REQUIRE(ctx->vol_layout == TOMO_VOLUME_PLANAR, "the fused gradient step + momentum takes the planar volume: set TOMO_VOLUME_PLANAR first");
     a.xt = xt_dev; a.xt_out = xt_dev; a.xold = xold_x_dev; a.xout = xold_x_dev;
     a.s0 = l_inv; a.s1 = beta; a.nonneg = nonneg;
     a.zquad = ctx->res_layout == TOMO_RESIDUAL_ZQUAD;
@@ -1122,6 +1307,7 @@
     int rc = bp_prepare(ctx, subset, res_dev, a);
     if (rc != TOMO_OK) return rc;
     TOMO_REQUIRE(z_dev && x_dev && u_dev && zu_out_dev, "NULL volume pointer");
+    TOMO_REQUIRE(ctx->vol_layout == TOMO_VOLUME_PLANAR, "the ADMM z-update takes the planar volume: set TOMO_VOLUME_PLANAR first");
     a.xt = x_dev; a.xout = z_dev; a.xt_out = zu_out_dev; a.xold = u_dev;
     a.s0 = tau; a.s1 = rho; a.s2 = one_minus_alpha; a.s3 = alpha;
     a.nonneg = nonneg; a.relax_on = relax_on;
diff --git a/tomobar_amd/csrc/tomo_api.hip b/tomobar_amd/csrc/tomo_api.hip
--- a/tomobar_amd/csrc/tomo_api.hip
+++ b/tomobar_amd/csrc/tomo_api.hip
@@ -57,7 +57,7 @@
     int *slot = nullptr;
     bool ok = false;
     if (k == "bp") { slot = &g_variant_bp; ok = allowed({0}, {1, 2, 3}); }
-    else if (k == "fp") { slot = &g_variant_fp; ok = allowed({0}, {1, 2, 3, 4}); }
+    else if (k == "fp") { slot = &g_variant_fp; ok = allowed({0, 5}, {1, 2, 3, 4}); }
     else if (k == "pdtv") { slot = &g_variant_pdtv; ok = allowed({0, 22}, {1, 2, 3, 21, 31, 32}); }
     else if (k == "roftv") { slot = &g_variant_roftv; ok = allowed({0}, {1, 2, 3, 4}); }
 #if TOMO_DEV
diff --git a/tomobar_amd/csrc/tomo_common.h b/tomobar_amd/csrc/tomo_common.h
--- a/tomobar_amd/csrc/tomo_common.h
+++ b/tomobar_amd/csrc/tomo_common.h
@@ -42,6 +42,7 @@
     int wbound[4] = {0, 0, 0, 0};
     int wbound_wide[4] = {0, 0, 0, 0};
     int wbound16[4] = {0, 0, 0, 0};
+    int wbound_wide13[4] = {0, 0, 0, 0};
 };
 
 struct tomo_ctx {
@@ -62,6 +63,8 @@
     bool volT_valid = false;
     hipStream_t volT_stream = nullptr;
     std::string last_fp_path, last_bp_path;
+    bool volT_quad = false;
+    int vol_layout = 0;
     int res_layout = 0;
 };
 
diff --git a/tomobar_amd/methodsIR_CuPy.py b/tomobar_amd/methodsIR_CuPy.py
--- a/tomobar_amd/methodsIR_CuPy.py
+++ b/tomobar_amd/methodsIR_CuPy.py
@@ -208,7 +208,6 @@
 
         t = float32(1.0)
         X = x0
-        X_t = x0.clone()
         res = {}
         X_grad = self._new_vol() if has_prox else None
         X_prox = self._new_vol() if has_prox else None
@@ -216,9 +215,17 @@
         A.invalidate()
         zquad = not (use_ring or use_swls) and not getattr(A, "has_vertical_shift", False)
         A.set_residual_layout("zquad" if zquad else "planar")
+        vquad = (has_prox and zquad and self.slab is None and hasattr(A, "volume_zquad_ok")
+                 and A.residual_layout() == "zquad"
+                 and all(A.volume_zquad_ok(s if use_os else None) for s in range(self.OS_number)))
         n_sub_total = a["iterations"] * self.OS_number
         mon = _RunMonitor(self, "FISTA", a, x0, r)
         try:
+            if vquad:
+                A.set_volume_layout("zquad")
+                X_t = A.volume_to_zquad(x0)
+            else:
+                X_t = x0.clone()
             for it_no in range(a["iterations"]):
                 for sub_ind in range(self.OS_number):
                     sub = sub_ind if use_os else None
@@ -254,6 +261,8 @@
                     break
         finally:
             A.set_residual_layout("planar")
+            if vquad:
+                A.set_volume_layout("planar")
             A.invalidate()
         return self._finalise(X, a)
 
diff --git a/tomobar_amd/projector.py b/tomobar_amd/projector.py
--- a/tomobar_amd/projector.py
+++ b/tomobar_amd/projector.py
@@ -84,6 +84,7 @@
 
         self.nz, self.n = self.detectors_y, self.recon_size
         self._vshift = None
+        self._vol_zquad = False
         self.slab = None
         self.nu = self.detectors_x + 2 * self.detectors_x_pad
         self.na = self.angles_vec.size
@@ -280,9 +281,57 @@
             return res
         return res.permute(0, 3, 1, 2).reshape(-1, res.shape[1], res.shape[2])[: self.nz].contiguous()
 
+    def volume_zquad_ok(self, os_index=None) -> bool:
+        if self._vshift is not None or self._adjoint == "matched":
+            return False
+        return bool(self._lib.tomo_ctx_volume_zquad_ok(self._ctx, self._sub(os_index)))
+
+    def set_volume_layout(self, layout: str, require_ok: bool = True):
+        if layout == "zquad" and require_ok:
+            subs = [None] if self.ordsub_number == 1 else range(self.ordsub_number)
+            if not all(self.volume_zquad_ok(s) for s in subs):
+                raise ValueError("the quad-interleaved volume is not available for this geometry (volume_zquad_ok)")
+        self._chk(self._lib.tomo_ctx_set_volume_layout(self._ctx, L.VOLUME_LAYOUT[layout]))
+        self._vol_zquad = layout == "zquad"
+
+    def volume_layout(self) -> str:
+        code = self._lib.tomo_ctx_volume_layout(self._ctx)
+        return {v: k for k, v in L.VOLUME_LAYOUT.items()}[code]
+
+    def volume_buffer(self) -> torch.Tensor:
+        if self.volume_layout() == "planar":
+            return torch.empty(self.vol_shape(), dtype=torch.float32, device=self._device)
+        return torch.empty(((self.nz + 3) // 4, self.n, self.n, 4), dtype=torch.float32, device=self._device)
+
+    def _check_volume(self, vol, what="volume"):
+        want = int(self._lib.tomo_ctx_volume_elems(self._ctx))
+        quad = self.volume_layout() == "zquad"
+        if vol.numel() != want or (vol.dim() == 4) != quad or vol.dtype != torch.float32 or not vol.is_contiguous():
+            raise ValueError(f"{what} of {vol.numel()} elements / rank {vol.dim()} does not match the context's current "
+                             f"'{self.volume_layout()}' volume layout ({want} floats): take it from volume_buffer() after "
+                             "set_volume_layout()")
+
+    def volume_to_zquad(self, x, out=None) -> torch.Tensor:
+        if self.volume_layout() != "zquad":
+            raise ValueError("volume_to_zquad needs set_volume_layout('zquad')")
+        x = self._vol_in(x)
+        if out is None:
+            out = self.volume_buffer()
+        self._check_volume(out)
+        with torch.cuda.device(self._device):
+            self._chk(self._lib.tomo_volume_to_zquad(self._ctx, ops.ptr(x), ops.ptr(out), ops.stream_ptr(x)))
+        return out
+
+    def volume_as_planar(self, vol) -> torch.Tensor:
+        if vol.dim() == 3:
+            return vol
+        return vol.permute(0, 3, 1, 2).reshape(-1, self.n, self.n)[: self.nz].contiguous()
+
     def residual(self, vol, b, w, fidelity: str, os_index, out, gathered: int = 0, robust=None):
         if self._vshift is None:
             self._check_residual(out, os_index)
+        if self._vol_zquad:
+            self._check_volume(vol)
         if robust is not None:
             mode, delta = robust
             if self._vshift is not None:
@@ -351,6 +400,8 @@
                                                 r.numel(), ops.stream_ptr(r)))
 
     def momentum(self, x, x_old, x_t, beta):
+        if self._vol_zquad:
+            self._check_volume(x_t, "x_t")
         with torch.cuda.device(self._device):
             self._chk(self._lib.tomo_momentum_transposed(self._ctx, ops.ptr(x), ops.ptr(x_old), ops.ptr(x_t), float(beta),
                                                      ops.stream_ptr(x)))
@@ -361,6 +412,8 @@
     def grad_step(self, res, x_t, x_out, l_inv, nonneg, os_index):
         if self._vshift is None:
             self._check_residual(res, os_index)
+        if self._vol_zquad:
+            self._check_volume(x_t, "x_t")
         res = self._adjoint_in(res, os_index)
         with torch.cuda.device(self._device):
             self._chk(self._bp_name("tomo_bp3d_fista")(self._ctx, self._sub(os_index), ops.ptr(res), ops.ptr(x_t), ops.ptr(x_out),
```

New measurement: 0.7475 iterations/s, median of 6. 1.03x the previous value.
